# MaaniGhaffari/cvo-rgbd

Hardware: AMD Instinct MI355X
Metric: frame-pair registrations/sec (higher is better)
Workload: dtype f32; 1 GPU; BASELINE configs[1] shape: 64 distinct synthetic 10000x10000 RGB-D cloud pairs (xyz + 5-dim colour) per align_many call, cvo align() to convergence, clouds resident in HBM; points_fixed=10000, points_moving=10000, mode=cvo, batch=64

## Files before the change

cvo-rgbd_amd/csrc/cvo_capi.cpp:

```cpp
#include "cvo_internal.h"

using namespace cvo_dev;
using namespace cvo_impl;

namespace cvo_impl {

int fail(cvo_hip_ctx *ctx, int code, const char *msg)
{
    if (ctx) ctx->err = msg;
    return code;
}

static std::atomic<bool> g_engine_debug{false};
bool engine_debug_on() { return g_engine_debug.load(std::memory_order_relaxed); }

namespace {
struct OptDef {
    const char *key;
    const char *env;
    int env_kind;
    double env_value;
};
const OptDef kOptions[] = {
    {"graph_capture", "CVO_HIP_GRAPH", 1, 1.0},           {"no_graph", "CVO_HIP_NO_GRAPH", 1, 1.0},
    {"head_graphs", "CVO_HIP_RUN_GRAPHS", 1, 1.0},        {"head_mode", "CVO_HIP_NO_HEAD", 1, 0.0},
    {"resident_runs", "CVO_HIP_NO_RUN", 1, 0.0},          {"run_solvers_max", "CVO_HIP_RUN_G_MAX", 2, 0.0},
    {"run_candidates_max", "CVO_HIP_RUN_CAND", 2, 0.0},   {"run_timeout_ms", nullptr, 0, 0.0},
    {"run_fault", nullptr, 0, 0.0},                       {"merged_launches", "CVO_HIP_NO_MERGE", 1, 0.0},
    {"async_builds", "CVO_HIP_NO_ASYNC", 1, 0.0},         {"list_pass_blocks", "CVO_HIP_PROC_BLOCKS", 2, 0.0},
    {"post_debug", "CVO_HIP_POST_DEBUG", 1, 1.0},         {"mailbox_timeout_s", "CVO_HIP_MAILBOX_TIMEOUT_S", 2, 0.0},
    {"candidate_records", "CVO_HIP_NO_CAND", 1, 0.0},     {"sync_upload", "CVO_HIP_SYNC_UPLOAD", 1, 1.0},
    {"engine_debug", "CVO_HIP_ENGINE_DEBUG", 1, 1.0},     {"one_launch_hand_over", "CVO_HIP_NO_CLOUD_ONE", 1, 0.0},
    {"small_calls_alone", "CVO_HIP_NO_ALONE", 1, 0.0},    {"fused_groups", "CVO_HIP_NO_FUSE", 1, 0.0},
    {"engines", "CVO_HIP_ENGINES_FORCE", 2, 0.0},         {"list_init", "CVO_HIP_LIST_INIT", 2, 0.0},
    {"kept_pack", "CVO_HIP_NO_PACK", 1, 0.0},             {"list_margin", "CVO_HIP_LIST_MARGIN", 2, 0.0},
    {"final_mirror", "CVO_HIP_NO_FINAL_MIRROR", 1, 0.0},  {"twist_on_shared_gpu", "CVO_HIP_TWIST_ON_SHARED_GPU", 1, 1.0},
    {"comm_debug", "CVO_HIP_COMM_DEBUG", 1, 1.0},         {"wait_policy", "CVO_HIP_WAIT_POLICY", 2, 0.0},
    {"acvo_runs", "CVO_HIP_NO_ACVO_RUN", 1, 0.0},         {"tail_alone", "CVO_HIP_TAIL_ALONE", 2, 0.0},         {"side_builds", "CVO_HIP_SIDE", 1, 1.0},
    {"run_build_at", "CVO_HIP_RUN_BUILD_AT", 2, 0.0},         {"alone_max", "CVO_HIP_ALONE_MAX", 2, 0.0},
    {"narrow_merge", "CVO_HIP_NARROW_MERGE", 1, 1.0},     {"narrow_blocks", "CVO_HIP_NARROW_BLOCKS", 2, 0.0},
    {"engine_crowd", "CVO_HIP_ENGINE_CROWD", 2, 0.0},     {"engine_merge_max", "CVO_HIP_ENGINE_MERGE_MAX", 2, 0.0},
    {"matches_combine", nullptr, 0, 0.0},                 {"scan_chunk", nullptr, 0, 0.0},
    {"record_narrow", "CVO_HIP_NO_RECORD_NARROW", 1, 0.0}, {"list_stale_max", "CVO_HIP_LIST_STALE_MAX", 2, 0.0},
};
void env_defaults(cvo_hip_ctx *ctx)
{
    for (const OptDef &d : kOptions) {
        if (!d.env) continue;
        const char *e = getenv(d.env);
        if (!e) continue;
        (void)apply_option(ctx, d.key, d.env_kind == 1 ? d.env_value : atof(e));
    }
}
}

int apply_option(cvo_hip_ctx *ctx, const char *key, double v)
{
    auto is = [&](const char *k) { return std::strcmp(key, k) == 0; };
    const bool on = v != 0.0;
    CtxOptions &o = ctx->opt;
    if (is("graph_capture")) { ctx->use_graphs = on && !o.no_graph; if (!ctx->use_graphs) drop_graphs(ctx); }
    else if (is("no_graph")) { o.no_graph = on; if (on) { ctx->use_graphs = false; drop_graphs(ctx); } }
    else if (is("head_graphs")) ctx->head_graphs = on;
    else if (is("head_mode")) ctx->allow_head = on;
    else if (is("resident_runs")) ctx->allow_run = on;
    else if (is("run_solvers_max")) {
        int cus = 0;
        if (hipDeviceGetAttribute(&cus, hipDeviceAttributeMultiprocessorCount, ctx->device) != hipSuccess || cus <= 0) cus = RUN_G + 8;
        ctx->run_g_max = v > 0.0 ? std::max(8, std::min((int)RUN_G, (int)v)) : std::max(8, std::min((int)RUN_G, cus - 8));
    }
    else if (is("run_candidates_max")) { if (v < 0.0) return CVO_HIP_ERR_INVALID; o.run_cand = (int)v; }
    else if (is("run_timeout_ms")) { if (v < 0.0 || v > 6.0e4) return CVO_HIP_ERR_INVALID; o.run_timeout_ms = v; }
    else if (is("run_fault")) { if (v < 0.0) return CVO_HIP_ERR_INVALID; o.run_fault = (int)v; }
    else if (is("merged_launches")) ctx->allow_merge = on;
    else if (is("async_builds")) ctx->allow_async = ctx->allow_async_self = on;
    else if (is("list_pass_blocks")) {
        const int b = (int)v;
        if (b == 0) { ctx->proc_blocks_forced = false; ctx->proc_blocks = ctx->proc_blocks_default = PROC_BLOCKS; }
        else if (b == 64 || b == 128 || b == 256 || b == 512 || b == 1024) { ctx->proc_blocks = ctx->proc_blocks_default = b; ctx->proc_blocks_forced = true; }
        else return CVO_HIP_ERR_INVALID;
    }
    else if (is("post_debug")) o.post_debug = on;
    else if (is("mailbox_timeout_s")) { if (!(v > 0.0)) return CVO_HIP_ERR_INVALID; o.mailbox_timeout_s = v; }
    else if (is("candidate_records")) o.no_cand = !on;
    else if (is("sync_upload")) o.sync_upload = on;
    else if (is("engine_debug")) { o.engine_debug = on; if (on) g_engine_debug.store(true, std::memory_order_relaxed); }
    else if (is("one_launch_hand_over")) o.no_cloud_one = !on;
    else if (is("small_calls_alone")) o.no_alone = !on;
    else if (is("fused_groups")) o.no_fuse = !on;
    else if (is("engines")) { if (v < 0.0 || v > 8.0) return CVO_HIP_ERR_INVALID; o.engines_force = (int)v; }
    else if (is("list_init")) { if (v < 0.0) return CVO_HIP_ERR_INVALID; o.list_init = v; }
    else if (is("kept_pack")) o.no_pack = !on;
    else if (is("matches_combine")) o.matches_combine = on;
    else if (is("scan_chunk")) { if (v < 0.0 || v > (double)SCAN_CHUNK) return CVO_HIP_ERR_INVALID; o.scan_chunk = (int)v; }
    else if (is("list_margin")) { if (v > 4.0) return CVO_HIP_ERR_INVALID; o.list_margin = v < 0.0 ? -1.0f : (float)v; }
    else if (is("record_narrow")) o.record_narrow = on;
    else if (is("list_stale_max")) { if (!(v >= 1.0 && v <= 64.0)) return CVO_HIP_ERR_INVALID; o.list_stale_max = (float)v; }
    else if (is("final_mirror")) o.no_final_mirror = !on;
    else if (is("twist_on_shared_gpu")) o.twist_on_shared_gpu = on;
    else if (is("comm_debug")) o.comm_debug = on;
    else if (is("wait_policy")) { if (v < 0.0 || v > 2.0) return CVO_HIP_ERR_INVALID; o.wait_policy = (int)v; }
    else if (is("acvo_runs")) o.no_acvo_run = !on;
    else if (is("tail_alone")) { if (v < 0.0 || v > 32.0) return CVO_HIP_ERR_INVALID; o.tail_alone = (int)v; }
    else if (is("run_restart")) o.no_restart = !on;
    else if (is("side_builds")) o.no_side_builds = !on;
    else if (is("run_build_at")) { if (!(v > 0.0 && v <= 1.0)) return CVO_HIP_ERR_INVALID; o.run_build_at = (float)v; }
    else if (is("alone_max")) { if (v < 0.0 || v > 64.0) return CVO_HIP_ERR_INVALID; o.alone_max = (int)v; }
    else if (is("narrow_merge")) o.narrow_merge = on;
    else if (is("narrow_blocks")) { const int b = (int)v; if (b != 0 && b != 32 && b != 64) return CVO_HIP_ERR_INVALID; o.narrow_blocks = b; }
    else if (is("engine_crowd")) { if (v < 0.0) return CVO_HIP_ERR_INVALID; o.engine_crowd = (int)std::min(v, 1.0e6); }
    else if (is("engine_merge_max")) { if (v < 0.0 || v > 32.0) return CVO_HIP_ERR_INVALID; o.engine_merge_max = (int)v; }
    else return CVO_HIP_ERR_INVALID;
    return CVO_HIP_OK;
}

const char *params_problem(const cvo_hip_params &p)
{
    if (p.mode != CVO_HIP_MODE_CVO && p.mode != CVO_HIP_MODE_ACVO)
        return "params.mode must be CVO_HIP_MODE_CVO or CVO_HIP_MODE_ACVO (MATLAB: default_params() returns mode CVO)";
    if (p.max_iter < 0) return "params.max_iter < 0";
    const float pos[] = {p.ell_init, p.sigma, p.sp_thres, p.c, p.d, p.c_ell, p.c_sigma};
    const char *pos_name[] = {"ell_init", "sigma", "sp_thres", "c", "d", "c_ell", "c_sigma"};
    static thread_local char msg[96];
    for (int i = 0; i < 7; ++i)
        if (!(pos[i] > 0.0f) || !std::isfinite(pos[i])) {
            snprintf(msg, sizeof(msg), "params.%s must be positive and finite", pos_name[i]);
            return msg;
        }
    if (p.mode == CVO_HIP_MODE_ACVO && (!(p.c_sp_thres > 0.0f) || !std::isfinite(p.c_sp_thres)))
        return "params.c_sp_thres must be positive and finite";
    if (p.mode == CVO_HIP_MODE_ACVO && (!(p.ell_max_init > 0.0f) || !std::isfinite(p.ell_max_init) ||
                                        !(p.ell_min >= 0.0f) || !std::isfinite(p.dl_step)))
        return "params.ell_max_init / ell_min / dl_step out of range";
    const float fin[] = {p.min_step, p.eps, p.eps_2, p.color_scale, p.ell_min};
    for (float v : fin)
        if (!std::isfinite(v)) return "params: min_step, eps, eps_2, color_scale, ell_min must be finite";
    if (p.color_scale < 0.0f) return "params.color_scale < 0";
    return nullptr;
}

DevParams make_dev_params(const cvo_hip_params &p)
{
    DevParams d{};
    d.mode = p.mode;
    d.max_iter = p.max_iter;
    d.ell_init = p.ell_init;
    d.ell_min = p.ell_min;
    d.ell_max_init = p.ell_max_init;
    d.sp = p.sp_thres;
    d.c_sp = (p.mode == CVO_HIP_MODE_ACVO) ? p.c_sp_thres : p.sp_thres;
    d.c = p.c;
    d.d = p.d;
    d.c_ell = p.c_ell;
    d.min_step = p.min_step;
    d.eps = p.eps;
    d.eps_2 = p.eps_2;
    const float s2 = p.sigma * p.sigma;
    const float cs2 = p.c_sigma * p.c_sigma;
    d.log_sp_s2 = (float)std::log((double)(p.sp_thres / s2));
    d.tau_c = (float)(-2.0 * p.c_ell * p.c_ell *
                      (double)(float)std::log((double)(d.c_sp / p.c_sigma / p.c_sigma)));
    d.s2_d = (double)s2;
    d.cs2_d = (double)cs2;
    d.dl_step = p.dl_step;
    d.color_scale = p.color_scale;
    d.build_at = 0.7f;
    d.record_narrow = 1;
    d.list_stale_max = 3.0f;
    d.list_margin = 0.15f;
    return d;
}


}

extern "C" {


const char *cvo_hip_error_string(int status)
{
    switch (status) {
    case CVO_HIP_OK: return "ok";
    case CVO_HIP_ERR_INVALID: return "invalid argument or call order";
    case CVO_HIP_ERR_HIP: return "HIP runtime error";
    case CVO_HIP_ERR_NOMEM: return "out of memory";
    case CVO_HIP_ERR_COMM: return "RCCL / all-reduce error";
    case CVO_HIP_ERR_NODEVICE: return "no usable HIP device";
    case CVO_HIP_ERR_RUN: return "a resident run timed out and the registration could not be redone";
    default: return "unknown status";
    }
}

const char *cvo_hip_last_error(const cvo_hip_ctx *ctx) { return ctx ? ctx->err.c_str() : ""; }

int cvo_hip_device_count(int *count)
{
    if (!count) return CVO_HIP_ERR_INVALID;
    int n = 0;
    if (hipGetDeviceCount(&n) != hipSuccess) n = 0;
    *count = n;
    return CVO_HIP_OK;
}

int cvo_hip_default_params(int mode, cvo_hip_params *p)
{
    if (!p || (mode != CVO_HIP_MODE_CVO && mode != CVO_HIP_MODE_ACVO && mode != CVO_HIP_MODE_MATLAB))
        return CVO_HIP_ERR_INVALID;
    std::memset(p, 0, sizeof(*p));
    p->mode = mode == CVO_HIP_MODE_MATLAB ? CVO_HIP_MODE_CVO : mode;
    p->max_iter = 2000;
    p->sigma = 0.1f;
    p->c = 7.0f;
    p->d = 7.0f;
    p->c_sigma = 1.0f;
    p->min_step = (float)(2 * 1.0e-1);
    p->eps = (float)(5 * 1.0e-5);
    p->eps_2 = (float)1.0e-5;
    if (mode == CVO_HIP_MODE_ACVO) {
        p->ell_init = 0.1f;
        p->ell_min = 0.0391f;
        p->ell_max_init = 0.15f;
        p->sp_thres = 8.315e-3f;
        p->c_sp_thres = 8.315e-3f;
        p->c_ell = 0.5f;
        p->dl_step = 0.3;
    } else {
        p->ell_init = 0.15f;
        p->ell_min = 0.0f;
        p->ell_max_init = 0.15f;
        p->sp_thres = 8e-3f;
        p->c_sp_thres = 8e-3f;
        p->c_ell = 200.0f;
        p->dl_step = 0.0;
    }
    if (mode == CVO_HIP_MODE_MATLAB) {
        p->sp_thres = 1e-3f;
        p->c_sp_thres = 1e-3f;
        p->eps = 5e-4f;
        p->eps_2 = 1e-4f;
        p->color_scale = 1e-5f;
    }
    return CVO_HIP_OK;
}

int cvo_hip_init_state(const cvo_hip_params *p, cvo_hip_state *s)
{
    if (!p || !s) return CVO_HIP_ERR_INVALID;
    std::memset(s, 0, sizeof(*s));
    s->R[0] = s->R[4] = s->R[8] = 1.0f;
    s->ell = p->ell_init;
    s->ell_max = p->ell_max_init;
    for (float *m : {s->transform, s->prev_transform, s->accum_transform})
        m[0] = m[5] = m[10] = m[15] = 1.0f;
    return CVO_HIP_OK;
}

// ... 449 lines not shown
    if (!ctx || !out) return CVO_HIP_ERR_INVALID;
    HIP_TRY(ctx, hipSetDevice(ctx->device));
    const bool had_tf = ctx->have_tf;
    std::swap(ctx->fixed, ctx->scratch_a);
    std::swap(ctx->moving, ctx->scratch_b);
    int rc = upload_cloud(ctx, ctx->fixed, xyz_a, feat_a, na, feat_layout);
    if (!rc) rc = upload_cloud(ctx, ctx->moving, xyz_b, feat_b, nb, feat_layout);
    if (!rc) rc = cvo_hip_function_inner_product(ctx, ell, out);
    std::swap(ctx->fixed, ctx->scratch_a);
    std::swap(ctx->moving, ctx->scratch_b);
    ctx->have_tf = had_tf;
    return rc;
}

int cvo_hip_get_wave_load(cvo_hip_ctx *ctx, uint32_t *members_per_wave, int capacity, int *waves)
{
    cvo_lock::Api api_guard;
    if (!ctx || !members_per_wave || !waves || capacity < 0) return CVO_HIP_ERR_INVALID;
    HIP_TRY(ctx, hipSetDevice(ctx->device));
    const int n = std::min(capacity, 4 * ctx->proc_blocks);
    *waves = 0;
    if (!ctx->kept_cnt.p || n <= 0) return CVO_HIP_OK;
    HIP_TRY(ctx, hipStreamSynchronize(ctx->stream));
    HIP_TRY(ctx, hipMemcpy(members_per_wave, ctx->kept_cnt.p, (size_t)n * sizeof(uint32_t), hipMemcpyDeviceToHost));
    *waves = n;
    return CVO_HIP_OK;
}

int cvo_hip_set_graph_capture(cvo_hip_ctx *ctx, int enable)
{
    cvo_lock::Api api_guard;
    if (!ctx) return CVO_HIP_ERR_INVALID;
    return apply_option(ctx, "graph_capture", enable ? 1.0 : 0.0);
}

int cvo_hip_set_profiling(cvo_hip_ctx *ctx, int enable)
{
    cvo_lock::Api api_guard;
    if (!ctx) return CVO_HIP_ERR_INVALID;
    ctx->profiling = enable != 0;
    return CVO_HIP_OK;
}

int cvo_hip_get_profile(cvo_hip_ctx *ctx, cvo_hip_profile *out, int reset)
{
    cvo_lock::Api api_guard;
    if (!ctx || !out) return CVO_HIP_ERR_INVALID;
    int rc = drain_events(ctx);
    if (rc) return rc;
    *out = ctx->prof;
    if (reset) ctx->prof = cvo_hip_profile{};
    return CVO_HIP_OK;
}

int cvo_hip_get_graph_stats(const cvo_hip_ctx *ctx, long long *launches_from_cache, long long *captures)
{
    if (!ctx || !launches_from_cache || !captures) return CVO_HIP_ERR_INVALID;
    *launches_from_cache = ctx->plans.hits;
    *captures = ctx->plans.captures;
    return CVO_HIP_OK;
}

int cvo_hip_get_run_stats(cvo_hip_ctx *ctx, int *runs, int *declined, int *iterations, int *candidates)
{
    cvo_lock::Api api_guard;
    if (!ctx || !ctx->st) return CVO_HIP_ERR_INVALID;
    struct { int32_t run_count, run_entered, run_iterations, run_candidates; } f{};
    static_assert(offsetof(DevState, run_candidates) - offsetof(DevState, run_count) == 12, "four consecutive words");
    if (hipSetDevice(ctx->device) != hipSuccess || hipStreamSynchronize(ctx->stream) != hipSuccess ||
        hipMemcpy(&f, reinterpret_cast<const char *>(ctx->st) + offsetof(DevState, run_count), sizeof(f), hipMemcpyDeviceToHost) != hipSuccess)
        return CVO_HIP_ERR_HIP;
    if (runs) *runs = f.run_entered;
    if (declined) *declined = f.run_count - f.run_entered;
    if (iterations) *iterations = f.run_iterations;
    if (candidates) *candidates = f.run_candidates;
    return CVO_HIP_OK;
}

int cvo_hip_get_list_stats(const cvo_hip_ctx *ctx, int *builds, int *narrowings, int *reexpansions)
{
    if (!ctx) return CVO_HIP_ERR_INVALID;
    if (builds) *builds = ctx->list_stats[0];
    if (narrowings) *narrowings = ctx->list_stats[1];
    if (reexpansions) *reexpansions = ctx->list_stats[2];
    return CVO_HIP_OK;
}

int cvo_hip_get_run_clocks(cvo_hip_ctx *ctx, long long clocks16[16])
{
    cvo_lock::Api api_guard;
    if (!ctx || !ctx->st || !clocks16) return CVO_HIP_ERR_INVALID;
    long long clk[16];
    static_assert(sizeof(clk) == sizeof(DevState::run_clk), "run_clk");
    if (hipSetDevice(ctx->device) != hipSuccess || hipStreamSynchronize(ctx->stream) != hipSuccess ||
        hipMemcpy(clk, reinterpret_cast<const char *>(ctx->st) + offsetof(DevState, run_clk), sizeof(clk), hipMemcpyDeviceToHost) != hipSuccess)
        return CVO_HIP_ERR_HIP;
    for (int q = 0; q < 16; ++q) clocks16[q] = clk[q];
    return CVO_HIP_OK;
}

int cvo_hip_set_option(cvo_hip_ctx *ctx, const char *key, double value)
{
    cvo_lock::Api api_guard;
    if (!ctx || !key) return CVO_HIP_ERR_INVALID;
    if (hipSetDevice(ctx->device) != hipSuccess) return CVO_HIP_ERR_HIP;
    const int rc = apply_option(ctx, key, value);
    if (rc) return fail(ctx, rc, "cvo_hip_set_option: unknown key or value out of range");
    return CVO_HIP_OK;
}

int cvo_hip_get_option(const cvo_hip_ctx *ctx, const char *key, double *value)
{
    if (!ctx || !key || !value) return CVO_HIP_ERR_INVALID;
    auto is = [&](const char *k) { return std::strcmp(key, k) == 0; };
    const CtxOptions &o = ctx->opt;
    if (is("graph_capture")) *value = ctx->use_graphs;
    else if (is("no_graph")) *value = o.no_graph;
    else if (is("head_graphs")) *value = ctx->head_graphs;
    else if (is("head_mode")) *value = ctx->allow_head;
    else if (is("resident_runs")) *value = ctx->allow_run;
    else if (is("run_solvers_max")) *value = ctx->run_g_max;
    else if (is("run_candidates_max")) *value = o.run_cand;
    else if (is("run_timeout_ms")) *value = o.run_timeout_ms;
    else if (is("run_fault")) *value = o.run_fault;
    else if (is("merged_launches")) *value = ctx->allow_merge;
    else if (is("async_builds")) *value = ctx->allow_async;
    else if (is("list_pass_blocks")) *value = ctx->proc_blocks_forced ? ctx->proc_blocks : 0;
    else if (is("post_debug")) *value = o.post_debug;
    else if (is("mailbox_timeout_s")) *value = o.mailbox_timeout_s;
    else if (is("candidate_records")) *value = !o.no_cand;
    else if (is("sync_upload")) *value = o.sync_upload;
    else if (is("engine_debug")) *value = o.engine_debug;
    else if (is("one_launch_hand_over")) *value = !o.no_cloud_one;
    else if (is("small_calls_alone")) *value = !o.no_alone;
    else if (is("fused_groups")) *value = !o.no_fuse;
    else if (is("engines")) *value = o.engines_force;
    else if (is("narrow_merge")) *value = o.narrow_merge;
    else if (is("narrow_blocks")) *value = o.narrow_blocks;
    else if (is("engine_crowd")) *value = o.engine_crowd;
    else if (is("engine_merge_max")) *value = o.engine_merge_max;
    else if (is("list_init")) *value = o.list_init;
    else if (is("kept_pack")) *value = !o.no_pack;
    else if (is("matches_combine")) *value = o.matches_combine;
    else if (is("scan_chunk")) *value = o.scan_chunk;
    else if (is("list_margin")) *value = o.list_margin;
    else if (is("record_narrow")) *value = o.record_narrow;
    else if (is("list_stale_max")) *value = o.list_stale_max;
    else if (is("final_mirror")) *value = !o.no_final_mirror;
    else if (is("twist_on_shared_gpu")) *value = o.twist_on_shared_gpu;
    else if (is("comm_debug")) *value = o.comm_debug;
    else if (is("wait_policy")) *value = o.wait_policy;
    else if (is("acvo_runs")) *value = !o.no_acvo_run;
    else if (is("tail_alone")) *value = o.tail_alone;
    else if (is("tail_handovers")) *value = (double)ctx->tail_handovers;
    else if (is("run_restart")) *value = !o.no_restart;
    else if (is("side_builds")) *value = !o.no_side_builds;
    else if (is("run_build_at")) *value = o.run_build_at;
    else if (is("side_builds_launched")) *value = (double)ctx->side_builds_launched;
    else if (is("alone_max")) *value = o.alone_max;
    else if (is("run_timeouts")) *value = (double)ctx->run_timeouts;
    else if (is("list_grows")) *value = (double)ctx->list_grows;
    else if (is("async_builds_named")) *value = (double)ctx->async_stats[0];
    else if (is("async_stalls")) *value = (double)ctx->async_stats[1];
    else if (is("run_aborts")) *value = (double)ctx->run_aborts;
    else if (is("engine_begins")) *value = (double)ctx->engine_begins;
    else if (is("engine_final_mirrored")) *value = (double)ctx->engine_final_mirrored;
    else if (is("engine_final_copied")) *value = (double)ctx->engine_final_copied;
    else if (is("no_run_backoff")) *value = ctx->no_run_backoff;
    else return CVO_HIP_ERR_INVALID;
    return CVO_HIP_OK;
}

long long cvo_hip_get_mirror_retries(void) { return mirror_retries().load(std::memory_order_relaxed); }

int cvo_hip_synchronize(cvo_hip_ctx *ctx)
{
    cvo_lock::Api api_guard;
    if (!ctx) return CVO_HIP_ERR_INVALID;
    HIP_TRY(ctx, hipStreamSynchronize(ctx->stream));
    return CVO_HIP_OK;
}


}
```

cvo-rgbd_amd/csrc/cvo_device.h:

```cpp
#pragma once

#include <hip/hip_runtime.h>
#include <hip/hip_ext.h>
#include <stddef.h>
#include <stdint.h>

#include "cvo_hip.h"
#include "se3_math.hpp"

namespace cvo_dev {

constexpr int FEAT_STRIDE = 8;
constexpr int FEAT_INDEX_SLOT = 5;

constexpr int BLOCK = 256;
constexpr int TILES_PER_WAVE = 4;
constexpr int ROWS_PER_WAVE = 16 * TILES_PER_WAVE;
constexpr int ROWS_PER_TILE = 4 * ROWS_PER_WAVE;
constexpr float PAD_BIG = 1.0e30f;
constexpr int PROC_BLOCKS = 1024;
constexpr int PROC_WAVES = PROC_BLOCKS * 4;

constexpr int NSUB = 256;
constexpr int PROC_PARTS = PROC_BLOCKS / NSUB;
constexpr int TILE_STAGE = 128;
constexpr int DEAL_SHIFT = 2;
constexpr int PAIR_QUEUE = 128;
constexpr int SEG = 64;
constexpr int MAX_CSEG = 32;

typedef uint4 TileEntry;

enum ProcMode { PROC_FLOW = 0, PROC_STEP = 1, PROC_SELF = 2 };
enum ListId { LIST_XY = 0, LIST_XX = 1, LIST_YY = 2, LIST_KEPT = 3, LIST_XYB = 4, LIST_XXB = 5, LIST_YYB = 6,
              LIST_N = 7 };
CVO_HD int self_list_id(int l, int buf) { return buf ? LIST_XXB + l : LIST_XX + l; }

constexpr int NACC_FLOW = 9;
constexpr int NACC_STEP = 4;
constexpr int NACC_SELF = 2;
constexpr int NACC_MAX = 9;

constexpr int RED_FLOW = 0, RED_XX = 9, RED_YY = 11, RED_STEP = 13, RED_N = 17;

enum { RUNNING = 0, DONE_BREAK_A = 1, DONE_BREAK_B = 2, DONE_MAX_ITER = 3, NEED_BIGGER_LIST = 4,
       DONE_COMM_ERROR = 5,
       DONE_RUN_TIMEOUT = 6 };

constexpr int MAX_WORLD = 16;
constexpr int MAIL_VALS = 14;
struct alignas(128) MailSlot {
    double v[MAIL_VALS];
    unsigned long long seq;
    unsigned long long pad_;
};
struct Mailbox {
    MailSlot slot[2][MAX_WORLD];
    unsigned long long owner_dev;
    unsigned long long pad_[15];
};
struct CommTable {
    Mailbox *peer[MAX_WORLD];
    int rank, world;
    long long timeout_ticks;
};

constexpr int RUN_G = 248;
constexpr int RUN_G_SMALL = 32;
constexpr int RUN_BLOCK = 512;
constexpr int RUN_WAVES = RUN_BLOCK / 64;
constexpr int RUN_LANES = RUN_G * RUN_BLOCK;
constexpr int RUN_R = 8;
constexpr int RUN_MIRROR_ABORTED = 1 << 29;
constexpr int RUN_MIRROR_ENTERED = 1 << 30;
constexpr int RUN_L = 8;
constexpr int RUN_CAP = RUN_LANES * (RUN_R + RUN_L);
constexpr unsigned RUN_LDS_BYTES = (unsigned)RUN_L * 2u * (unsigned)RUN_BLOCK * 16u;
constexpr int RUN_NV = 13;
#ifndef CVO_RUN_A
#define CVO_RUN_A 4
#endif
constexpr int RUN_A = CVO_RUN_A;
constexpr int RUN_GEN = 4;
constexpr int RUN_CHAINS = 8;
struct RunMail {
    unsigned long long w[RUN_GEN][RUN_G + 1][2 * RUN_NV];
    unsigned long long p[RUN_GEN][RUN_CHAINS][2 * RUN_NV];
    unsigned long long entry_ticket;
    unsigned long long entry_go;
    unsigned long long side_done;
    unsigned long long side_req;
};
constexpr int RUN_G_SIDE = 128;

struct KernConsts {
    float tau;
    float tau_c;
    float sp;
    float inv_c;
    float inv_d;
    float inv_l3;
    float cb, cg, cd;
    float cscale;
    double s2_d;
    double cs2_d;
    double ninv_2l2;
    double ninv_2cl2;
};

struct DevParams {
    int32_t mode, max_iter;
    float ell_init, ell_min, ell_max_init;
    float sp, c_sp;
    float c, d, c_ell;
    float min_step, eps, eps_2;
    float log_sp_s2;
    float tau_c;
    float list_margin;
    int32_t async_xy;
    float build_at;
    int32_t async_self;
    float color_scale;
    float run_cand_cap;
    int32_t record_narrow;
    float list_stale_max;
    double s2_d, cs2_d, dl_step;
};

struct alignas(16) DevHead {
    float R[9], T[3];
    float ell, ell_max;
    float Rt[9], t[3];
    float used_Rt[9], used_t[3];
    KernConsts kc;
    float kc_ell, kc_pad_;
    float center[3];
    float xmax, y0max;
    float tauf[3];
    int32_t n_fixed;
    uint32_t pad0_;
    float list_r[3];
    int32_t list_ok[3];
    int32_t reuse[3];
    int32_t ck_nblk[3];
    float list_Rt[9], list_t[3];
    float rec_r;
    int32_t narrow;
    float rec_Rt[9], rec_t[3];
    int32_t list_stat[3];
    int32_t async_stat[2];
    int32_t rec_pad_;
    int32_t xy_active, xy_target, stall, xy_fresh;
    int32_t xy_ok[2];
    int32_t xy_ck[2];
    float xy_r[2];
    float tauf_build;
    float r_last;
    float xy_Rt[2][9], xy_t[2][3];
    int32_t sf_active[2], sf_target[2], sf_fresh[2];
    int32_t sf_ok[2][2];
    int32_t sf_ck[2][2];
    float sf_r[2][2];
    float sf_tauf_build[2];
    cvo_math::XiConsts xi;
    float omega[3], v[3];
    double dl;
    double red[RED_N];
    int32_t k;
    int32_t done;
    int32_t iter;
    int32_t n_exec;
    int32_t n_slots;
    int32_t pending;
    unsigned long long mail_snap;
    int32_t run_hint;
    int32_t head_check_;
    int32_t rec_count[2];
};
enum { REC_NARROW = 1, REC_BOUNDED = 2 };
CVO_HD unsigned head_check_mix(unsigned x, unsigned y, unsigned z, unsigned w, unsigned piece)
{
    return (x * 0x9E3779B1u + y * 0x85EBCA77u + z * 0xC2B2AE3Du + w * 0x27D4EB2Fu) ^ (piece * 0x165667B1u + 0x9E3779B9u);
}
struct DevState : DevHead {
    uint32_t sub[LIST_N][NSUB];
    uint32_t ovf[2][8];
    uint32_t built[3][64];
    int32_t run_count;
    int32_t run_entered;
    int32_t run_iterations;
    int32_t run_candidates;
    int32_t run_last_entered, run_last_aborted;
    long long run_clk[16];
    unsigned long long mail_seq;
    unsigned long long run_seq;
};
static_assert(LIST_N <= 8, "DevState::ovf holds 8 lists");
constexpr size_t DEVSTATE_INIT_BYTES = offsetof(DevState, mail_seq);
constexpr size_t DEVSTATE_HEAD_BYTES = sizeof(DevHead);
static_assert(offsetof(DevState, sub) == sizeof(DevHead) && sizeof(DevHead) % 16 == 0, "the tail follows the head");

constexpr int MAXG = 16;
template <class A> struct Grp { A a[MAXG]; };
constexpr int ENGINE_SLOTS = 32;

struct FilterArgs {
    const float4 *pos_a;
    const float4 *pos_b;
    const float4 *seg_a;
    const float4 *seg_b;
    DevState *st;
    DevState *st2;
    TileEntry *tiles;
    TileEntry *tiles_b;
    int async_xy;
    uint32_t subcap;
    int list;
    int row_lo, row_hi;
    int nb;
    int jt;
    int tf_a, tf_b;
    int check_done;
    int gx, gy;
    long long *dbg;
    float4 *pos_bt;
};

struct ProcessArgs {
    const float4 *pos_a;
    const float *feat_a;
    const float4 *pos_b;
    const float *feat_b;
    const TileEntry *tiles;
    const TileEntry *tiles_b;
    int async_xy;
    int async_self;
    uint2 *kept_ij;
    float *kept_a;
    uint32_t *kept_cnt;
    double *partials;
    DevState *st;
    DevState *st2;
    uint32_t subcap;
    uint32_t kept_wcap;
    int nblk;
    const double *flow_part;
    const double *xx_part;
    const double *yy_part;
    cvo_hip_trace *trace; int trace_cap;
    int acvo;
    int32_t *done_mirror;
    int list;
    int row_hi, nb;
    int first_counted;
    int tf_a, tf_b;
    int check_done;
    int weight;
    uint2 *cand;
    uint32_t *cand_cnt;
    uint2 *cand_b;
    uint32_t *cand_cnt_b;
    int need_d2;
    const CommTable *comm;
    int kept_packed;
    unsigned kept_ebase;
};

enum { POST_REDUCE = 1, POST_MATH = 2 };

struct PostFlowArgs {
    DevState *st;
    const double *part_flow;
    const double *part_xx;
    const double *part_yy;
    cvo_hip_trace *trace; int trace_cap;
    int flags;
    int check_done;
    int32_t *done_mirror;
    int nblk;
    const CommTable *comm;
    DevParams prm;
};

struct PostStepArgs {
    DevState *st;
    DevState *st2;
    const double *part_step;
    cvo_hip_trace *trace; int trace_cap;
    int flags;
    int check_done;
    long long *dbg;
    int32_t *done_mirror;
    int ck_nblk[3];
    int32_t *progress_mirror;
    int nblk;
    const CommTable *comm;
    DevHead *final_mirror;
    uint32_t *build_mask;
    uint32_t slot_bit;
    RunMail *run_mail;
    int32_t *run_mirror;
    int32_t *hint_mirror;
    int run_iters;
    int run_g_max;
    long long run_timeout_ticks;
    int32_t *side_mirror;
    float run_build_at;
    int run_fault;
    DevParams prm;
};

constexpr size_t kTableHeaderBytes = 256;
constexpr int MAX_OPS = 10;
struct OpArgs {
    ProcessArgs p;
    FilterArgs f;
    union {
        PostFlowArgs pf;
        PostStepArgs ps;
    };
    int np, n0, n1, n2;
};
struct Slot {
    int active;
    int pad_[3];
    OpArgs op[MAX_OPS];
};

CVO_HD KernConsts make_kconsts(const DevParams &p, float ell)
{
    KernConsts k;
    const float l = ell;
    k.tau = (float)(-2.0 * l * l * (double)p.log_sp_s2);
    k.tau_c = p.tau_c;
    k.sp = p.sp;
    k.inv_c = 1 / p.c;
    k.inv_d = 1 / p.d;
    const float ell_3 = l * l * l;
    k.inv_l3 = 1 / ell_3;
    const float temp_coef = (float)(1 / (2.0 * l * l));
    k.cb = (float)(-2.0 * temp_coef);
    k.cg = -temp_coef;
    k.cd = (float)(2.0 * temp_coef);
    k.cscale = p.color_scale;
    if (k.cscale > 0.0f) k.tau = (float)((double)k.tau * 1.00001);
    if (!(k.tau > 0.0f)) k.tau = 0.0f;
    k.s2_d = p.s2_d;
    k.cs2_d = p.cs2_d;
    k.ninv_2l2 = -1.0 / (2.0 * l * l);
    k.ninv_2cl2 = -1.0 / (2.0 * p.c_ell * p.c_ell);
    return k;
}

CVO_HD void compute_filter_bounds(DevHead *s, bool identity)
{
    float ymax = s->y0max;
    if (!identity) {
        const float *R = s->R, *c = s->center;
        float sh2 = 0.0f;
        for (int r = 0; r < 3; ++r) {
            const float rc = R[3 * r] * c[0] + R[3 * r + 1] * c[1] + R[3 * r + 2] * c[2];
            const float d = s->T[r] + rc - c[r];
            sh2 += d * d;
        }
        ymax = (s->y0max + sqrtf(sh2)) * 1.0001f + 1e-6f;
    }
    const float u16 = 16.0f / 16777216.0f;
    const float sxy = (s->xmax + ymax) * (s->xmax + ymax);
    const float sxx = 4.0f * s->xmax * s->xmax;
    const float syy = 4.0f * ymax * ymax;
    const float tau = s->kc.tau;
    s->tauf[LIST_XY] = (tau + u16 * sxy) * 1.000001f;
    s->tauf[LIST_XX] = (tau + u16 * sxx) * 1.000001f;
    s->tauf[LIST_YY] = (tau + u16 * syy) * 1.000001f;
}

CVO_HD bool spheres_near(const float4 sa, const float4 sb, float reach)
{
    const float ex = sa.x - sb.x, ey = sa.y - sb.y, ez = sa.z - sb.z;
    const float d2 = __builtin_fmaf(ez, ez, __builtin_fmaf(ey, ey, ex * ex));
    const float rr = (sa.w + sb.w + reach) * 1.00001f + 1e-5f;
    return d2 * 0.99999f <= rr * rr;
}
CVO_HD float cull_slack(const float *t, const float cx, const float cy, const float cz, const float xmax, const float y0max)
{
    const float W = ((fabsf(cx) + fabsf(cy)) + fabsf(cz)) + (xmax + y0max);
    return (64.0f / 16777216.0f) * (3.0003f * W + ((fabsf(t[0]) + fabsf(t[1])) + fabsf(t[2])));
}

CVO_HD float reuse_slack(const float *t, const float *c, const float xmax, const float y0max, const float sides)
{
    const float W = ((fabsf(c[0]) + fabsf(c[1])) + fabsf(c[2])) + (xmax + y0max);
    const float S = 3.0003f * W + ((fabsf(t[0]) + fabsf(t[1])) + fabsf(t[2]));
    return 1.0e-4f * (1.0f + xmax + y0max) + sides * (22.0f / 16777216.0f) * S;
}

constexpr float LIST_LOOSE = 1.3f;
CVO_HD float pose_travel(const DevHead *s, const float *Rt0, const float *t0, const float ymax)
{
    float f2 = 0.0f, c2 = 0.0f;
    for (int r = 0; r < 3; ++r) {
        float dc = s->t[r] - t0[r];
        for (int q = 0; q < 3; ++q) {
            const float d = s->Rt[3 * r + q] - Rt0[3 * r + q];
            f2 += d * d;
            dc += d * s->center[q];
        }
        c2 += dc * dc;
    }
    return sqrtf(0.5f * f2) * 1.001f * ymax + sqrtf(c2);
}
CVO_HD void plan_lists(DevHead *s, DevHead *bulk, const bool store, const DevParams &p, const float r_now)
{
    const float ymax = s->y0max;
    const float slack_xx = reuse_slack(s->t, s->center, s->xmax, ymax, 0.0f), slack_xy = reuse_slack(s->t, s->center, s->xmax, ymax, 1.0f);
    const float wide_yy = slack_xy - slack_xx;
    const float margin = p.list_margin;
    const bool sync_xy = s->list_ok[LIST_XY] && !p.async_xy;
    const float travel = sync_xy ? pose_travel(s, s->list_Rt, s->list_t, ymax) : 0.0f;
#pragma unroll
    for (int l = 0; l < 3; ++l) {
        if (l == LIST_XY && p.async_xy) continue;
        if (l != LIST_XY && p.async_self) continue;
        if (l != LIST_XY && p.mode != CVO_HIP_MODE_ACVO) { s->reuse[l] = 1; continue; }
        const float slack = l == LIST_XX ? slack_xx : slack_xy;
        const float need = (r_now + (l == LIST_XY ? travel : 0.0f)) * 1.0001f + slack;
        const float lr = s->list_r[l];
        const float r0 = r_now * 1.0001f + slack;
        const float rb = r0 * (1.0f + margin);
        bool keep = margin > 0.0f && s->list_ok[l] && need <= lr;
        if (l == LIST_XY && p.record_narrow && keep && s->ck_nblk[LIST_XY] != 0) {
            const float tr = pose_travel(s, s->rec_Rt, s->rec_t, ymax);
            const float rr = s->rec_r;
            keep = (r_now + tr) * 1.0001f + slack <= rr && lr <= fmaxf(p.list_stale_max, LIST_LOOSE) * (1.0f + margin) * r0;
            s->narrow &= REC_BOUNDED;
            if (keep && !(rr <= LIST_LOOSE * (1.0f + margin) * r0)) {
                keep = (rb + tr) * 1.0001f + slack <= rr;
                if (keep) {
                    s->rec_r = rb * 1.000001f;
                    s->narrow = REC_NARROW | REC_BOUNDED;
                    s->list_stat[1] += 1;
                    if (store) {
                        for (int q = 0; q < 9; ++q) bulk->rec_Rt[q] = s->Rt[q];
                        for (int q = 0; q < 3; ++q) bulk->rec_t[q] = s->t[q];
                    }
                }
            }
        } else {
            keep = keep && lr <= LIST_LOOSE * (1.0f + margin) * r0;
            if (l == LIST_XY) s->narrow &= REC_BOUNDED;
        }
        s->reuse[l] = keep ? 1 : 0;
        if (keep) continue;
        s->ck_nblk[l] = 0;
        s->list_r[l] = rb * 1.000001f;
        s->list_ok[l] = 1;
        if (margin > 0.0f) {
            const float rw = s->list_r[l] + (l == LIST_YY ? wide_yy : 0.0f);
            s->tauf[l] = (rw * rw + (s->tauf[l] - s->kc.tau)) * 1.000001f;
        }
        if (l == LIST_XY) {
            s->rec_r = s->list_r[l];
            s->narrow = p.record_narrow ? REC_BOUNDED : 0;
            s->list_stat[0] += 1;
            if (store) {
                for (int q = 0; q < 9; ++q) bulk->list_Rt[q] = bulk->rec_Rt[q] = s->Rt[q];
                for (int q = 0; q < 3; ++q) bulk->list_t[q] = bulk->rec_t[q] = s->t[q];
            }
        }
    }
}

template <int B> CVO_HD float xy_travel(const DevHead *s, const DevHead *rec)
{
    float f2 = 0.0f, c2 = 0.0f;
    for (int r = 0; r < 3; ++r) {
        float dc = s->t[r] - rec->xy_t[B][r];
        for (int q = 0; q < 3; ++q) {
// ... 469 lines not shown
```

cvo-rgbd_amd/csrc/cvo_engine.cpp:

```cpp
#include "cvo_internal.h"

using namespace cvo_dev;
using namespace cvo_impl;

namespace cvo_impl {

bool fusable(const cvo_hip_ctx *c) { return !c->profiling && !multi_rank(c) && !(c->prm.color_scale > 0.0f); }



struct EngineProfile {
    std::mutex mu;
    bool on = false;
    double flow_ms = 0.0, flow_slots = 0.0;
    long long flow_launches = 0;
    std::vector<float> dur_us, period_us;
    std::vector<int> slots;
};
EngineProfile *engine_profile()
{
    static EngineProfile *p = new EngineProfile;
    return p;
}

bool better_alone(const std::deque<AlignJob *> &pending)
{
    const bool off = !pending.empty() && pending.front()->ctx->opt.no_alone;
    if (off || engine_profile()->on) return false;
    double pairs = 0.0;
    bool acvo = false;
    for (const AlignJob *j : pending) {
        const cvo_hip_ctx *c = j->ctx;
        acvo = c->prm.mode == CVO_HIP_MODE_ACVO;
        if (!c->allow_head || !c->allow_async || !c->allow_merge || c->opt.no_cand || c->fixed.np > 65536 || c->moving.np > 65536 ||
            (acvo ? !c->allow_async_self : !c->allow_run))
            return false;
        pairs = std::max(pairs, (double)c->fixed.n * (double)c->moving.n);
    }
    const size_t few = acvo ? (pairs <= 1.6e7 ? 12 : (pairs <= 5.0e7 ? 4 : (pairs <= 1.2e8 ? 4 : 0)))
                            : (pairs <= 1.6e7 ? 12 : (pairs <= 5.0e7 ? 8 : (pairs <= 2.0e8 ? 4 : 0)));
    if (const int force = pending.front()->ctx->opt.alone_max) return pending.size() <= (size_t)force;
    return pending.size() <= few;
}

struct Engine {
    int device = 0;
    hipStream_t s = nullptr;
    TableBuf tab;
    PlanCache plans;
    bool in_use = false;

    AlignJob *member[ENGINE_SLOTS] = {};
    std::vector<RecOp> ops[ENGINE_SLOTS];
    Slot slot[ENGINE_SLOTS];
    struct Retire { hipEvent_t ev = nullptr; std::vector<AlignJob *> jobs; };
    std::vector<Retire> retiring;
    hipEvent_t ev[4] = {};
    std::vector<PrepareEntry> prep;
    long long launched = 0, checked = 0;
    int zdim = 0;
    bool crowded = true, use_graph = true, dirty = true, failed = false;
    int batch_len = kEngineBatch;
    bool narrow = false;
    bool narrow_merge = false;
    int narrow_blocks = 0;
    bool wind_down = false;
    std::vector<TLaunch> plan;
    struct FlowEv { hipEvent_t a, b; int live; };
    std::vector<FlowEv> flow_ev;
    long long n_batches[5] = {}, n_replans = 0, n_inserts = 0, n_sends = 0, n_prepares = 0, n_mirrored = 0, n_copied = 0;
    double t_replan = 0, t_insert = 0, t_launch = 0, t_finish = 0, t_wait = 0, t_collect = 0, t_idle_at = 0;
    static double now_ms() { return std::chrono::duration<double, std::milli>(std::chrono::steady_clock::now().time_since_epoch()).count(); }

    int create(int dev)
    {
        device = dev;
        if (hipSetDevice(dev) != hipSuccess) return -1;
        if (hipStreamCreateWithFlags(&s, hipStreamNonBlocking) != hipSuccess) return -1;
        if (tab.init(ENGINE_SLOTS, s) != 0) return -1;
        for (auto &e : ev)
            if (hipEventCreateWithFlags(&e, hipEventDisableTiming) != hipSuccess) return -1;
        return 0;
    }

    int live() const { int n = 0; for (AlignJob *j : member) n += j != nullptr; return n; }
    bool idle() const { return live() == 0 && retiring.empty() && launched == checked; }

    static int nblk_for(int z)
    {
        constexpr int budget = 2048;
        int nblk = 64;
        while (nblk < PROC_BLOCKS && nblk * 2 <= (budget + z / 2) / std::max(1, z)) nblk *= 2;
        return nblk;
    }

    void finish_job(AlignJob *j, int rc)
    {
        j->rc = rc;
        j->phase = 2;
        j->in_group = false;
        j->ctx->loop_stream = nullptr;
        j->ctx->crowded = false;
        j->ctx->lone = true;
        j->ctx->proc_blocks = j->ctx->proc_blocks_default;
    }

    void fail_all(const char *msg, std::deque<AlignJob *> &pending)
    {
        failed = true;
        (void)hipStreamSynchronize(s);
        for (AlignJob *&j : member)
            if (j) { finish_job(j, fail(j->ctx, CVO_HIP_ERR_HIP, msg)); j = nullptr; }
        for (auto &r : retiring) {
            for (AlignJob *j : r.jobs) finish_job(j, fail(j->ctx, CVO_HIP_ERR_HIP, msg));
            if (r.ev) (void)hipEventDestroy(r.ev);
        }
        retiring.clear();
        for (AlignJob *j : pending) { j->rc = fail(j->ctx, CVO_HIP_ERR_HIP, msg); j->phase = 2; }
        pending.clear();
        prep.clear();
        for (int z = 0; z < ENGINE_SLOTS; ++z) slot[z].active = 0;
        (void)tab.sync(slot, s, 0);
        (void)hipStreamSynchronize(s);
        launched = checked = 0;
    }

    int flush_prepare()
    {
        if (prep.empty()) return CVO_HIP_OK;
        launch_prepare_many(prep.data(), (int)prep.size(), s, tab.masks());
        n_prepares += ((long long)prep.size() + MAXG - 1) / MAXG;
        prep.clear();
        return hipGetLastError() == hipSuccess ? CVO_HIP_OK : CVO_HIP_ERR_HIP;
    }

    int insert(AlignJob *j, int z)
    {
        cvo_hip_ctx *c = j->ctx;
        c->loop_stream = s;
        c->crowded = crowded;
        c->lone = false;
        j->in_group = true;
        int rc = CVO_HIP_OK;
        if (j->phase == 3) {
            int32_t zero = 0;
            std::memcpy(&c->st_host[kPollSlots].done, &zero, sizeof(zero));
            if (hipMemcpyAsync(reinterpret_cast<char *>(c->st) + offsetof(DevState, done), &c->st_host[kPollSlots].done,
                               sizeof(zero), hipMemcpyHostToDevice, s) != hipSuccess)
                rc = fail(c, CVO_HIP_ERR_HIP, "resume failed");
            *c->done_mirror = 0;
            PrepareEntry e{};
            e.st = c->st;
            e.prm = loop_params(c);
            if (!rc) prep.push_back(e);
            j->phase = 0;
        } else {
            PrepareEntry e{};
            rc = job_begin(*j, &e);
            if (!rc) prep.push_back(e);
        }
        if (rc) { finish_job(j, rc); return rc; }
        ++c->engine_begins;
        if (j->phase != 0) {
            Retire r;
            if (flush_prepare() != CVO_HIP_OK ||
                hipMemcpyAsync(&c->st_host[0], c->st, sizeof(DevState), hipMemcpyDeviceToHost, s) != hipSuccess ||
                hipEventCreateWithFlags(&r.ev, hipEventDisableTiming) != hipSuccess || hipEventRecord(r.ev, s) != hipSuccess) {
                if (r.ev) (void)hipEventDestroy(r.ev);
                finish_job(j, fail(c, CVO_HIP_ERR_HIP, "event failed"));
                return CVO_HIP_ERR_HIP;
            }
            r.jobs.push_back(j);
            retiring.push_back(r);
            return CVO_HIP_OK;
        }
        member[z] = j;
        ops[z].clear();
        dirty = true;
        return CVO_HIP_OK;
    }

    int replan()
    {
        int n = 0;
        for (int z = 0; z < ENGINE_SLOTS; ++z) n += member[z] != nullptr;
        int zd = 1;
        while (zd < n) zd *= 2;
        if (n > 16 && n <= 24) zd = 24;
        for (int z = ENGINE_SLOTS - 1, hole = 0; z >= zd; --z) {
            if (!member[z]) continue;
            while (member[hole]) ++hole;
            member[hole] = member[z]; member[z] = nullptr;
            ops[hole].swap(ops[z]); ops[z].clear();
        }
        const bool regeom = zd != zdim;
        zdim = zd;
        const int nblk = (narrow && narrow_blocks > 0) ? std::min(narrow_blocks, nblk_for(zdim)) : nblk_for(zdim);
        int merge_max = 2;
        std::vector<const std::vector<RecOp> *> po;
        std::vector<Slot *> ps;
        for (int z = 0; z < ENGINE_SLOTS; ++z)
            if (member[z]) { merge_max = member[z]->ctx->opt.engine_merge_max; break; }
        for (int z = 0; z < ENGINE_SLOTS; ++z) {
            if (!member[z]) { slot[z].active = 0; continue; }
            cvo_hip_ctx *c = member[z]->ctx;
            if (regeom || ops[z].empty()) {
                c->proc_blocks = nblk;
                const bool allow = c->allow_merge;
                if (zdim > merge_max && !(narrow && narrow_merge)) c->allow_merge = false;
                const int rc = record_iteration(c, ops[z], 0);
                c->allow_merge = allow;
                if (rc) return rc;
            }
            std::memset(&slot[z], 0, sizeof(Slot));
            slot[z].active = 1;
            po.push_back(&ops[z]);
            ps.push_back(&slot[z]);
        }
        if (!plan_fused(po, ps, zdim, plan)) return CVO_HIP_ERR_INVALID;
        for (int z = 0; z < ENGINE_SLOTS; ++z)
            if (member[z]) set_build_masks(slot[z], plan, tab.masks(), z);
        const int nq = po.empty() ? 0 : (int)po[0]->size();
        if (tab.sync(slot, s, nq) != 0) return CVO_HIP_ERR_HIP;
        ++n_replans;
        dirty = false;
        return CVO_HIP_OK;
    }

    void collect_stopped()
    {
        Retire r;
        for (int z = 0; z < ENGINE_SLOTS; ++z) {
            AlignJob *j = member[z];
            if (!j) continue;
            cvo_hip_ctx *c = j->ctx;
            const int32_t verdict = *(volatile int32_t *)c->done_mirror;
            if (verdict == RUNNING) continue;
            const bool mirrored = (verdict == DONE_BREAK_A || verdict == DONE_BREAK_B || verdict == DONE_MAX_ITER) && c->final_mirror &&
                                  !c->opt.no_final_mirror && !multi_rank(c);
            if (mirrored && take_final_mirror(c, verdict)) {
                ++n_mirrored;
                ++c->engine_final_mirrored;
                finish_job(j, job_finish(*j));
            } else if (hipMemcpyAsync(&j->ctx->st_host[0], j->ctx->st, sizeof(DevState), hipMemcpyDeviceToHost, s) != hipSuccess) {
                finish_job(j, fail(j->ctx, CVO_HIP_ERR_HIP, "state copy failed"));
            } else {
                ++n_copied;
                ++c->engine_final_copied;
                r.jobs.push_back(j);
            }
            member[z] = nullptr;
            ops[z].clear();
            dirty = true;
        }
        if (r.jobs.empty()) return;
        if (hipEventCreateWithFlags(&r.ev, hipEventDisableTiming) != hipSuccess || hipEventRecord(r.ev, s) != hipSuccess) {
            for (AlignJob *j : r.jobs) finish_job(j, fail(j->ctx, CVO_HIP_ERR_HIP, "event failed"));
            if (r.ev) (void)hipEventDestroy(r.ev);
            return;
        }
        retiring.push_back(r);
    }

    bool finish_arrived(std::deque<AlignJob *> &pending, bool block)
    {
        bool moved = false;
        while (!retiring.empty()) {
            Retire &r = retiring.front();
            const hipError_t q = block ? hipEventSynchronize(r.ev) : hipEventQuery(r.ev);
            if (q == hipErrorNotReady) break;
            block = false;
            for (AlignJob *j : r.jobs) {
                cvo_hip_ctx *c = j->ctx;
                const DevState &cur = c->st_host[0];
                if (q != hipSuccess) { finish_job(j, fail(c, CVO_HIP_ERR_HIP, "state event failed")); continue; }
                if (cur.done != NEED_BIGGER_LIST) { finish_job(j, job_finish(*j)); continue; }
                int rc = CVO_HIP_OK;
                for (int l = 0; l < LIST_N && !rc; ++l)
                    if (cur.ovf[0][l] | cur.ovf[1][l]) {
                        uint32_t worst = 0;
                        for (int qq = 0; qq < NSUB; ++qq) worst = std::max(worst, cur.sub[l][qq]);
                        const double grown = std::min(
                            4.0e9, std::max((double)worst * NSUB, (double)c->lists[l].cap) * 1.5 + 1024.0);
                        rc = ensure_list(c, l, 0, 0, grown);
                        ++c->list_grows;
                    }
                for (int qq = 0; qq < 3 && !rc; ++qq) {
                    const int la = qq == 0 ? LIST_XY : (qq == 1 ? LIST_XX : LIST_YY), lb = qq == 0 ? LIST_XYB : (qq == 1 ? LIST_XXB : LIST_YYB);
                    if (!c->lists[la].cap && !c->lists[lb].cap) continue;
                    const double both = (double)std::max(c->lists[la].cap, c->lists[lb].cap);
                    rc = ensure_list(c, la, 0, 0, both);
                    if (!rc && c->lists[lb].cap) rc = ensure_list(c, lb, 0, 0, both);
                }
                if (rc) { finish_job(j, rc); continue; }
                j->executed_base = cur.k;
                j->phase = 3;
                pending.push_front(j);
            }
            (void)hipEventDestroy(r.ev);
            retiring.erase(retiring.begin());
            moved = true;
        }
        return moved;
    }

    int launch_one_batch()
    {
        const int batch = batch_len;
        if (engine_profile()->on) {
            for (int k = 0; k < batch; ++k)
                for (const TLaunch &l : plan) {
                    if (l.kernel == TK_FLOW || l.kernel == TK_FLOW_D2) {
                        FlowEv fe{nullptr, nullptr, live()};
                        if (hipEventCreate(&fe.a) == hipSuccess && hipEventCreate(&fe.b) == hipSuccess) {
                            launch_table(tab.dev, l, s, fe.a, fe.b);
                            flow_ev.push_back(fe);
                            continue;
                        }
                    }
                    launch_table(tab.dev, l, s);
                }
            return hipGetLastError() == hipSuccess ? CVO_HIP_OK : CVO_HIP_ERR_HIP;
        }
        return run_plan(tab.dev, plans, plan, s, use_graph, batch);
    }

    bool pump(std::deque<AlignJob *> &pending, int want)
    {
        if (failed) return false;
        if (hipSetDevice(device) != hipSuccess) { fail_all("hipSetDevice failed", pending); return true; }
        bool moved = false;
        while (checked < launched) {
            const hipError_t q = hipEventQuery(ev[checked % 4]);
            if (q == hipErrorNotReady) break;
            if (q != hipSuccess) { fail_all("fused poll failed", pending); return true; }
            ++checked;
            { const double t0 = now_ms(); collect_stopped(); t_collect += now_ms() - t0; }
            moved = true;
        }
        { const double t0 = now_ms(); if (finish_arrived(pending, false)) moved = true; t_finish += now_ms() - t0; }
        while (!wind_down && !pending.empty() && live() < std::min(want, (int)ENGINE_SLOTS)) {
            AlignJob *j = pending.front();
            pending.pop_front();
            int z = 0;
            while (member[z]) ++z;
            { const double t0 = now_ms(); insert(j, z); t_insert += now_ms() - t0; }
            moved = true;
        }
        {
            const double t0 = now_ms();
            const int rc = flush_prepare();
            t_insert += now_ms() - t0;
            if (rc) { fail_all("prepare launch failed", pending); return true; }
        }
        constexpr long long depth = 2;
        while (live() > 0 && launched - checked < depth && !wind_down) {
            if (dirty) {
                const double t0 = now_ms();
                const int rc = replan();
                t_replan += now_ms() - t0;
                if (rc) { fail_all("fused launch recording failed", pending); return true; }
            }
            const double t_l0 = now_ms();
            const int rc_launch = launch_one_batch();
            if (rc_launch != CVO_HIP_OK ||
                hipEventRecord(ev[launched % 4], s) != hipSuccess) {
                fail_all("fused launch failed", pending);
                return true;
            }
            t_launch += now_ms() - t_l0;
            ++launched;
            ++n_batches[zdim >= 16 ? 4 : (zdim >= 8 ? 3 : (zdim >= 4 ? 2 : (zdim >= 2 ? 1 : 0)))];
            moved = true;
        }
        if (live() == 0 && dirty && launched == checked) {
            if (replan() != CVO_HIP_OK) { fail_all("table update failed", pending); return true; }
        }
        return moved;
    }

    void release_members(std::vector<AlignJob *> &out)
    {
        if (!wind_down || launched != checked || failed) return;
        collect_stopped();
        for (int z = 0; z < ENGINE_SLOTS; ++z) {
            AlignJob *j = member[z];
            if (!j) continue;
            out.push_back(j);
            member[z] = nullptr;
            ops[z].clear();
            dirty = true;
        }
    }

    void wait_oldest(std::deque<AlignJob *> &pending)
    {
        const double t0 = now_ms();
        struct Acc { double &t; double t0; ~Acc() { t += now_ms() - t0; } } acc{t_wait, t0};
        if (checked < launched) {
            if (hipEventSynchronize(ev[checked % 4]) != hipSuccess) fail_all("fused poll failed", pending);
        } else if (!retiring.empty()) {
            (void)hipEventSynchronize(retiring.front().ev);
        }
    }
};

std::mutex *engine_mutex()
{
    static std::mutex *mu = new std::mutex;
    return mu;
}

Engine *engine_checkout(int device)
{
    static std::vector<Engine *> *all = new std::vector<Engine *>();
    std::lock_guard<std::mutex> lock(*engine_mutex());
    for (Engine *e : *all)
        if (!e->in_use && e->device == device && !e->failed) { e->in_use = true; return e; }
    size_t have = 0;
    for (Engine *e : *all) have += e->device == device && !e->failed;
    Engine *first = nullptr;
    for (size_t k = have; k < std::max<size_t>(have + 1, 4); ++k) {
        Engine *e = new (std::nothrow) Engine();
        if (!e) break;
        if (e->create(device) != 0) { (void)hipGetLastError(); delete e; break; }
        all->push_back(e);
        if (!first) first = e;
    }
    if (first) first->in_use = true;
    return first;
}

void engine_release(Engine *e)
{
    if (!e->flow_ev.empty()) {
        EngineProfile *pr = engine_profile();
        std::lock_guard<std::mutex> plock(pr->mu);
        for (size_t q = 0; q < e->flow_ev.size(); ++q) {
            auto &fe = e->flow_ev[q];
            float ms = 0.f, gap = 0.f;
            if (hipEventSynchronize(fe.b) == hipSuccess && hipEventElapsedTime(&ms, fe.a, fe.b) == hipSuccess) {
                pr->flow_ms += ms; pr->flow_launches++; pr->flow_slots += fe.live;
                if (q + 1 < e->flow_ev.size() && hipEventElapsedTime(&gap, fe.a, e->flow_ev[q + 1].a) != hipSuccess) gap = 0.f;
                if (pr->dur_us.size() < (size_t)1 << 20) {
                    pr->dur_us.push_back(ms * 1e3f); pr->period_us.push_back(gap * 1e3f); pr->slots.push_back(fe.live);
                }
            }
        }
        for (auto &fe : e->flow_ev) {
            (void)hipEventDestroy(fe.a);
            (void)hipEventDestroy(fe.b);
        }
        e->flow_ev.clear();
    }
    std::lock_guard<std::mutex> lock(*engine_mutex());
    if (engine_debug_on())
        fprintf(stderr, "[cvo_hip] engine %p: batches at zdim 1/2/4/8/16: %lld %lld %lld %lld %lld, replans %lld, "
                "prepare launches %lld, final states mirrored %lld copied %lld, graph captures %lld hits %lld; host ms: insert %.2f replan %.2f launch %.2f collect %.2f finish %.2f wait %.2f\n",
                (void *)e, e->n_batches[0], e->n_batches[1], e->n_batches[2],
                e->n_batches[3], e->n_batches[4], e->n_replans, e->n_prepares, e->n_mirrored, e->n_copied, e->plans.captures, e->plans.hits,
                e->t_insert, e->t_replan, e->t_launch, e->t_collect, e->t_finish, e->t_wait);
    e->t_insert = e->t_replan = e->t_launch = e->t_collect = e->t_finish = e->t_wait = 0;
    for (long long &v : e->n_batches) v = 0;
    e->n_replans = e->n_prepares = e->n_mirrored = e->n_copied = 0;
    e->launched = e->checked = 0;
    e->in_use = false;
}


}

extern "C" {

int cvo_hip_align_many(cvo_hip_ctx **ctxs, cvo_hip_state **states, int *n_iters, int count)
{
    cvo_lock::Api api_guard;
    if (count < 0 || (count > 0 && (!ctxs || !states))) return CVO_HIP_ERR_INVALID;
    const bool dbg_many = engine_debug_on();
    const double t_many0 = Engine::now_ms();
    struct Tell { double t0; int n; ~Tell() { if (engine_debug_on()) fprintf(stderr, "[cvo_hip] align_many(%d): %.2f ms\n", n, Engine::now_ms() - t0); } } tell{t_many0, count};
    std::vector<AlignJob> jobs((size_t)count);
    for (int i = 0; i < count; ++i) {
        if (!ctxs[i] || !states[i]) return CVO_HIP_ERR_INVALID;
        for (int k = 0; k < i; ++k)
            if (ctxs[k] == ctxs[i]) return CVO_HIP_ERR_INVALID;
        jobs[i].ctx = ctxs[i];
        jobs[i].s = states[i];
        jobs[i].n_iter = n_iters ? &n_iters[i] : nullptr;
    }
    int first_err = CVO_HIP_OK;
    std::vector<char> taken((size_t)count, 0);
    std::vector<AlignJob *> leavers;
    const bool no_fuse = count > 0 && ctxs[0] && ctxs[0]->opt.no_fuse;
    if (!no_fuse && count > 1) {
        constexpr int gmax = ENGINE_SLOTS;
        for (int i = 0; i < count; ++i) {
            if (taken[i] || jobs[i].phase != 0 || !fusable(jobs[i].ctx)) continue;
            std::deque<AlignJob *> pending;
            for (int k = i; k < count; ++k)
                if (!taken[k] && jobs[k].phase == 0 && fusable(jobs[k].ctx) &&
                    jobs[k].ctx->device == jobs[i].ctx->device &&
                    jobs[k].ctx->prm.mode == jobs[i].ctx->prm.mode)
                    pending.push_back(&jobs[k]);
            if (pending.size() < 2) continue;
            if (better_alone(pending)) continue;
            for (AlignJob *j : pending) taken[j - &jobs[0]] = 1;
            const size_t total = pending.size();
            constexpr size_t max_engines = 4;
            size_t ngroups = total > 3 * ENGINE_SLOTS ? 4 : (total >= 40 ? 3 : (total >= 8 ? 2 : 1));
            ngroups = std::max<size_t>(1, std::min(ngroups, max_engines));
            if (const int force = pending.front()->ctx->opt.engines_force) ngroups = (size_t)std::max(1, std::min(force, 8));
            bool graphs_ok = true;
            for (AlignJob *j : pending) graphs_ok = graphs_ok && j->ctx->use_graphs;
            const int crowd = pending.front()->ctx->opt.engine_crowd;
            std::vector<Engine *> engines;
            for (size_t g = 0; g < ngroups; ++g) {
                Engine *e = engine_checkout(jobs[i].ctx->device);
                if (!e) break;
                e->crowded = (int)total > crowd;
                e->use_graph = graphs_ok;
                e->zdim = 0;
                e->wind_down = false;
                e->narrow = false;
                e->narrow_merge = pending.front()->ctx->opt.narrow_merge;
                e->narrow_blocks = pending.front()->ctx->opt.narrow_blocks;
                e->batch_len = kEngineBatch;
                e->t_idle_at = 0;
                e->dirty = true;
                engines.push_back(e);
            }
            if (engines.empty()) {
                for (AlignJob *j : pending) taken[j - &jobs[0]] = 0;
                continue;
            }
            const int share = std::min<int>(gmax, (int)((total + engines.size() - 1) / engines.size()));
            const int tail_k = pending.empty() ? 0 : pending.front()->ctx->opt.tail_alone;
            const int narrow_from = pending.empty() ? 0 : (pending.front()->ctx->prm.mode == CVO_HIP_MODE_ACVO ? 8 : 24);
            bool tail_ok = tail_k > 0 && !engine_profile()->on;
            for (AlignJob *j : pending) {
                const cvo_hip_ctx *c = j->ctx;
                tail_ok = tail_ok && c->allow_head && c->allow_async && c->allow_merge && !c->opt.no_cand && runs_allowed(c) && c->fixed.np <= 65536 &&
                          c->moving.np <= 65536 && (c->prm.mode == CVO_HIP_MODE_CVO || (c->allow_async_self && !c->opt.no_acvo_run)) &&
                          (double)c->fixed.n * (double)c->moving.n <= 2.0e8;
            }
            const bool narrow_merge_ok = !pending.empty() && (pending.front()->ctx->opt.narrow_merge || pending.front()->ctx->opt.narrow_blocks > 0) && !engine_profile()->on;
            int dbg_left = -1, dbg_narrow = -1;
            for (;;) {
                bool any = false, moved = false;
                if ((tail_ok || narrow_merge_ok) && pending.empty() && !engines.front()->wind_down) {
                    int left = 0;
                    bool narrow = true, settled = true;
                    for (Engine *e : engines) {
                        settled = settled && e->retiring.empty();
                        for (AlignJob *j : e->member)
                            if (j) { ++left; narrow = narrow && *(volatile int32_t *)j->ctx->progress_mirror >= narrow_from; }
                    }
                    if (narrow_merge_ok && narrow && left > 0 && !engines.front()->narrow)
                        for (Engine *e : engines) {
                            e->narrow = true;
                            e->dirty = true;
                            for (int z = 0; z < ENGINE_SLOTS; ++z) e->ops[z].clear();
                        }
                    if (dbg_many && (left != dbg_left || (int)narrow != dbg_narrow)) { dbg_left = left; dbg_narrow = (int)narrow; fprintf(stderr, "[cvo_hip]   %.2f ms: %d left (narrow %d settled %d)\n", Engine::now_ms() - t_many0, left, (int)narrow, (int)settled); }
                    (void)settled;
                    if (tail_ok && left > 0 && left <= tail_k && narrow) {
                        for (Engine *e : engines) e->wind_down = true;
                        if (dbg_many) {
                            fprintf(stderr, "[cvo_hip]   tail: %d registrations left after %.2f ms, slots done:", left, Engine::now_ms() - t_many0);
                            for (Engine *e : engines)
                                for (AlignJob *j : e->member)
                                    if (j) fprintf(stderr, " %d", *(volatile int32_t *)j->ctx->progress_mirror);
                            fprintf(stderr, "\n");
                        }
                    }
                }
                for (Engine *e : engines) {
                    if (e->wind_down) {
                        const size_t before = leavers.size();
                        e->release_members(leavers);
                        if (leavers.size() != before) {
                            moved = true;
                            if (dbg_many) fprintf(stderr, "[cvo_hip]   tail: %zu registrations leave engine %p after %.2f ms\n", leavers.size() - before, (void *)e, Engine::now_ms() - t_many0);
                        }
                        while (!pending.empty()) {
                            leavers.push_back(pending.front());
                            pending.pop_front();
                            moved = true;
                        }
                    }
                    if (e->pump(pending, share)) moved = true;
                    if (!e->idle()) any = true;
                    else if (dbg_many && e->t_idle_at == 0) {
                        e->t_idle_at = Engine::now_ms();
                        fprintf(stderr, "[cvo_hip]   engine %p idle after %.2f ms\n", (void *)e, e->t_idle_at - t_many0);
                    }
                }
                if (!any && pending.empty()) break;
                bool alive = false;
                for (Engine *e : engines) alive = alive || !e->failed;
                if (!alive) break;
                if (!moved)
                    for (Engine *e : engines)
                        if (!e->idle() && !e->failed) { e->wait_oldest(pending); break; }
            }
            for (Engine *e : engines) { e->wind_down = false; e->narrow = false; e->batch_len = kEngineBatch; engine_release(e); }
        }
        for (int i = 0; i < count; ++i)
            if (jobs[i].phase == 2 && jobs[i].rc && !first_err) first_err = jobs[i].rc;
    }
    std::vector<char> cont((size_t)count, 0);
    for (AlignJob *j : leavers) {
        const size_t i = (size_t)(j - &jobs[0]);
        taken[i] = 0;
        cont[i] = 1;
    }
    int k_alone = 0;
    for (int i = 0; i < count; ++i)
        if (!taken[i] && jobs[i].phase != 2) ++k_alone;
    const int kAloneLive = std::max<int>(8, (int)leavers.size());
    std::vector<char> begun((size_t)count, 0);
    auto begin_job = [&](int i) {
        int cus = 0;
        if (hipDeviceGetAttribute(&cus, hipDeviceAttributeMultiprocessorCount, jobs[i].ctx->device) != hipSuccess || cus <= 0) cus = RUN_G + 8;
        const int share = std::min(k_alone, kAloneLive);
        jobs[i].ctx->run_g_call = share > 1 ? std::max(8, (cus - 8) / share - 1) : RUN_G;
        jobs[i].ctx->call_no_spec = share > 2;
        jobs[i].ctx->crowded = false;
        jobs[i].ctx->lone = true;
        jobs[i].paced_nb = true;
        begun[(size_t)i] = 1;
        const int rc = cont[(size_t)i] ? job_continue_alone(jobs[i]) : job_begin(jobs[i]);
        if (rc) { jobs[i].rc = rc; jobs[i].phase = 2; if (!first_err) first_err = rc; }
    };
    auto is_alone = [&](int i) { return !taken[i]; };
    for (;;) {
        int live = 0, moved = 0, first_live = -1, waiting = 0;
        for (int i = 0; i < count; ++i)
            if (is_alone(i) && begun[(size_t)i] && jobs[i].phase != 2) ++live;
        for (int i = 0; i < count; ++i)
            if (is_alone(i) && !begun[(size_t)i] && jobs[i].phase != 2 && (live < kAloneLive || multi_rank(jobs[i].ctx))) {
                begin_job(i); ++moved;
                if (jobs[i].phase != 2) ++live;
            }
        live = 0;
        for (int i = 0; i < count; ++i) {
            if (jobs[i].phase == 2) continue;
            if (is_alone(i) && !begun[(size_t)i]) { ++waiting; continue; }
            const int before_phase = jobs[i].phase, before_checked = jobs[i].checked + jobs[i].batches;
            if (job_pump(jobs[i], false)) {
                if (jobs[i].rc && !first_err) first_err = jobs[i].rc;
                ++moved;
                continue;
            }
            ++live;
            if (first_live < 0) first_live = i;
            if (jobs[i].phase != before_phase || jobs[i].checked + jobs[i].batches != before_checked) ++moved;
        }
        if (live == 0 && waiting == 0) break;
        if (!moved && first_live >= 0) {
            if (job_pump(jobs[first_live], true) && jobs[first_live].rc && !first_err)
                first_err = jobs[first_live].rc;
        }
    }
    return first_err;
}

int cvo_hip_engine_profiling(int enable)
{
    EngineProfile *pr = engine_profile();
    std::lock_guard<std::mutex> lock(pr->mu);
    pr->on = enable != 0;
    return CVO_HIP_OK;
}

int cvo_hip_get_engine_profile(double *flow_ms, long long *flow_launches, double *flow_registrations, int reset)
{
    if (!flow_ms || !flow_launches || !flow_registrations) return CVO_HIP_ERR_INVALID;
    EngineProfile *pr = engine_profile();
    std::lock_guard<std::mutex> lock(pr->mu);
    *flow_ms = pr->flow_ms; *flow_launches = pr->flow_launches; *flow_registrations = pr->flow_slots;
    if (reset) { pr->flow_ms = 0.0; pr->flow_launches = 0; pr->flow_slots = 0.0; pr->dur_us.clear(); pr->period_us.clear(); pr->slots.clear(); }
    return CVO_HIP_OK;
}

int cvo_hip_get_engine_flow_trace(float *dur_us, float *period_us, int *slots, int capacity, int *count, int reset)
{
    if (!count || capacity < 0) return CVO_HIP_ERR_INVALID;
    EngineProfile *pr = engine_profile();
    std::lock_guard<std::mutex> lock(pr->mu);
    const int n = (int)std::min<size_t>(pr->dur_us.size(), (size_t)capacity);
    for (int q = 0; q < n; ++q) {
        if (dur_us) dur_us[q] = pr->dur_us[(size_t)q];
        if (period_us) period_us[q] = pr->period_us[(size_t)q];
        if (slots) slots[q] = pr->slots[(size_t)q];
    }
    *count = (int)pr->dur_us.size();
    if (reset) { pr->dur_us.clear(); pr->period_us.clear(); pr->slots.clear(); }
    return CVO_HIP_OK;
}


}
```

cvo-rgbd_amd/csrc/cvo_internal.h:

```cpp
#pragma once
#include "cvo_hip.h"

#include <hip/hip_runtime.h>

#include <algorithm>
#include <atomic>
#include <chrono>
#include <cmath>
#include <cstddef>
#include <cstdint>
#include <cstdio>
#include <cstdlib>
#include <cstring>
#include <deque>
#include <memory>
#include <mutex>
#include <new>
#include <string>
#include <thread>
#include <vector>

#include "cvo_cloud.h"
#include "cvo_comm.h"
#include "cvo_device.h"
// ... 39 lines not shown
};

struct FilterPlan {
    dim3 grid;
    int jt = 0;
};

struct DevBuf {
    void *p = nullptr;
    size_t bytes = 0;
};

struct PinBuf {
    void *p = nullptr;
    size_t bytes = 0;
};

struct List {
    DevBuf a, b;
    uint32_t cap = 0;
};

constexpr int kEngineBatch = 10;
constexpr int kBatch = 8;

constexpr int kStage = 4;
struct TableBuf {
    Slot *dev = nullptr;
    char *raw = nullptr;
    int nslots = 0;
    std::vector<Slot> image;
    Slot *stage = nullptr;
    hipEvent_t stage_ev[kStage] = {};
    bool stage_used[kStage] = {};
    int next = 0;

    int init(int n, hipStream_t s)
    {
        if (dev) return 0;
        if (hipMalloc((void **)&raw, kTableHeaderBytes + (size_t)n * sizeof(Slot)) != hipSuccess) { raw = nullptr; return -1; }
        dev = reinterpret_cast<Slot *>(raw + kTableHeaderBytes);
        if (hipMemsetAsync(raw, 0, kTableHeaderBytes + (size_t)n * sizeof(Slot), s) != hipSuccess) return -1;
        if (arm(s) != 0) return -1;
        if (hipHostMalloc((void **)&stage, (size_t)kStage * n * sizeof(Slot), hipHostMallocDefault) != hipSuccess) return -1;
        for (int i = 0; i < kStage; ++i)
            if (hipEventCreateWithFlags(&stage_ev[i], hipEventDisableTiming) != hipSuccess) return -1;
        nslots = n;
        image.assign((size_t)n, Slot{});
        return 0;
    }
    void destroy()
    {
        for (int i = 0; i < kStage; ++i)
            if (stage_ev[i]) (void)hipEventDestroy(stage_ev[i]);
        if (stage) (void)hipHostFree(stage);
        if (raw) (void)hipFree(raw);
        dev = nullptr; raw = nullptr; stage = nullptr; nslots = 0;
        image.clear();
    }
    uint32_t *masks() const { return reinterpret_cast<uint32_t *>(raw); }
    int arm(hipStream_t s) { return hipMemsetAsync(raw, 0xff, 4 * sizeof(uint32_t), s) == hipSuccess ? 0 : -1; }
    int sync(const Slot *want, hipStream_t s, int nq = MAX_OPS)
    {
        const size_t head = offsetof(Slot, op);
        int lo = nslots, hi = -1;
        for (int z = 0; z < nslots; ++z) {
            const Slot &img = image[(size_t)z];
            bool same = std::memcmp(&img, &want[z], head) == 0;
            if (same && want[z].active) same = std::memcmp(img.op, want[z].op, (size_t)nq * sizeof(OpArgs)) == 0;
            if (!same) { lo = std::min(lo, z); hi = z; }
        }
        if (hi < 0) return 0;
        const int b = next;
        next = (next + 1) % kStage;
        if (stage_used[b] && hipEventSynchronize(stage_ev[b]) != hipSuccess) return -1;
        Slot *st = stage + (size_t)b * nslots;
        const size_t n = (size_t)(hi - lo + 1);
        for (int z = lo; z <= hi; ++z) {
            if (want[z].active) image[(size_t)z] = want[z];
            else image[(size_t)z].active = 0;
            st[z] = image[(size_t)z];
        }
        if (hipMemcpyAsync(&dev[lo], &st[lo], n * sizeof(Slot), hipMemcpyHostToDevice, s) != hipSuccess) return -1;
        if (arm(s) != 0) return -1;
        if (hipEventRecord(stage_ev[b], s) != hipSuccess) return -1;
        stage_used[b] = true;
        return 0;
    }
};

struct PlanGraph {
    std::vector<TLaunch> pre;
    std::vector<TLaunch> plan;
    int iterations = 0;
    hipGraph_t graph = nullptr;
    hipGraphExec_t exec = nullptr;
    uint64_t stamp = 0;
};
struct PlanCache {
    std::vector<PlanGraph> graphs;
    uint64_t clock = 0;
    long long hits = 0, captures = 0;
    int fails = 0;
    void drop()
    {
        for (auto &g : graphs) {
            if (g.exec) (void)hipGraphExecDestroy(g.exec);
            if (g.graph) (void)hipGraphDestroy(g.graph);
        }
        graphs.clear();
    }
};
constexpr int kPollSlots = 4;
constexpr int kEvProcFlow = 10, kEvProcStep = 11;
constexpr int kProcStepTwist = 100;
constexpr int kFlowBuild = 101;
constexpr int kFilterAhead = 102;

struct RecOp {
    enum Kind { FILTER, PROCESS, POST_FLOW, POST_STEP } kind;
    int mode = 0;
    FilterArgs f{};
    ProcessArgs p{};
    PostFlowArgs pf{};
    PostStepArgs ps{};
};


}

using namespace cvo_dev;
using namespace cvo_impl;

struct CtxOptions {
    bool no_cand = false;
    bool no_graph = false;
    bool sync_upload = false;
    bool engine_debug = false;
    bool no_cloud_one = false;
    bool no_alone = false;
    bool no_fuse = false;
    bool no_pack = false;
    bool matches_combine = true;
    int scan_chunk = 0;
    bool no_final_mirror = false;
    bool twist_on_shared_gpu = false;
    bool comm_debug = false;
    bool post_debug = false;
    bool no_side_builds = true;
    float run_build_at = 0.6f;
    bool no_restart = false;
    bool no_acvo_run = false;
    int tail_alone = 8;
    int alone_max = 0;
    int engines_force = 0;
    int narrow_blocks = 0;
    bool narrow_merge = false;
    int engine_crowd = 2;
    int engine_merge_max = 2;
    double list_init = 0.0;
    float list_margin = -1.0f;
    bool record_narrow = true;
    float list_stale_max = 3.0f;
    int run_cand = 0;
    double mailbox_timeout_s = 5.0;
    double run_timeout_ms = 0.0;
    int run_fault = 0;
    int wait_policy = 0;
};

struct cvo_hip_ctx {
    CtxOptions opt;
    int no_run_backoff = 0;
    long long side_builds_launched = 0;
    long long tail_handovers = 0;
    long long engine_begins = 0;
    long long engine_final_mirrored = 0;
    long long engine_final_copied = 0;
    long long run_aborts = 0;
    int list_stats[3] = {0, 0, 0};
    int async_stats[2] = {0, 0};
    long long list_grows = 0;
    long long run_timeouts = 0;
    int device = 0;
    hipStream_t stream = nullptr;
    bool own_stream = false;
    cvo_hip_params prm{};
    DevParams dprm{};
    Cloud fixed, moving;
    Cloud scratch_a, scratch_b;
    DevState *st = nullptr;
    DevHead *st2 = nullptr;
    bool head_mode = false;
    bool allow_head = true;
    DevState *st_host = nullptr;
    int32_t *done_mirror = nullptr;
    int32_t *progress_mirror = nullptr;
    DevHead *final_mirror = nullptr;
    int32_t *run_mirror = nullptr;
    int32_t *hint_mirror = nullptr;
    int32_t *side_mirror = nullptr;
    hipStream_t side_stream = nullptr;
    std::vector<TLaunch> plan_side;
    DevBuf run_mail;
    bool plan_has_final_mirror = false;
    bool allow_run = true;
    int run_g_max = RUN_G;
    int run_g_call = RUN_G;
    bool call_no_spec = false;
    int big_run_backoff = 0;
    bool spec_first_run = true;
    bool head_graphs = false;
    int run_small_max = 0;
    int run_nnz_max = 0;
    std::vector<TLaunch> plan_pre;
    std::vector<RecOp> *rec = nullptr;
    int proc_blocks = PROC_BLOCKS;
    int proc_blocks_default = PROC_BLOCKS;
    bool proc_blocks_forced = false;
    DevBuf raw_xyz, raw_feat;
    DevBuf sort_keys[2], sort_idx[2], sort_tmp;
    float *bbox_dev = nullptr;
    float *bbox_host = nullptr;
    FilterArgs xy_build{};
    bool have_xy_build = false;
    bool allow_async = true;
    bool crowded = false;
    DevBuf cand[3], cand_cnt[3];
    DevBuf cand_xyb, cand_cnt_xyb;
    DevBuf cand_sfb[2], cand_cnt_sfb[2];
    int ck_nblk[3] = {0, 0, 0};
    DevBuf pos_bt;
    bool lone = true;
    bool allow_async_self = true;
    bool use_async_self = false;
    bool use_async = false;
    bool in_loop = false;
    bool plan_recording = false;
    bool merge_twist = false;
    bool allow_merge = true;
    cvo_hip_trace *cur_trace = nullptr;
    int cur_trace_cap = 0;
    hipEvent_t poll_ev[kPollSlots]{};
    DevBuf part_flow, part_xx, part_yy, part_step;
    DevBuf part_hess;
    DevBuf part_score;
    struct ScorePin *score_pin = nullptr;
    DevBuf part_matches;
    PinBuf match_stage;
    DevBuf scan_dev;
    PinBuf scan_stage;
    List lists[LIST_N];
    DevBuf kept_cnt;
    cvo_hip_trace *trace_dev = nullptr;
    int trace_dev_cap = 0;
    bool have_tf = false;
    int row_lo = 0, row_hi = -1, srow_lo = 0, srow_hi = -1;
    bool sharded = false;
    cvo_comm *comm = nullptr;
    Mailbox *mailbox = nullptr;
    CommTable *comm_table = nullptr;
    void *mail_opened[MAX_WORLD] = {};
    int mail_rank = 0, mail_world = 0;
    bool mail_shared_device = false;
    unsigned long long mail_dev_id = 0;
    bool mail_broken = false;
    cvo_hip_allreduce_fn user_allreduce = nullptr;
    void *user_allreduce_arg = nullptr;
    bool profiling = false;
    long long *post_dbg = nullptr;
    TableBuf table;
    PlanCache plans;
    std::vector<TLaunch> plan;
    hipStream_t loop_stream = nullptr;
    bool warm = false;
    bool use_graphs = true;
    int iter_tag = -1;
    std::vector<EventPair> events;
    cvo_hip_profile prof{};
    std::string err;
};

namespace cvo_impl {

#define HIP_TRY(ctx, expr)                                                                   \
    do {                                                                                     \
        hipError_t e_ = (expr);                                                              \
        if (e_ != hipSuccess) {                                                              \
            if (ctx) (ctx)->err = std::string(#expr) + ": " + hipGetErrorString(e_);         \
            return CVO_HIP_ERR_HIP;                                                          \
        }                                                                                    \
    } while (0)

struct AlignJob {
    cvo_hip_ctx *ctx = nullptr;
    cvo_hip_state *s = nullptr;
    cvo_hip_trace *trace = nullptr;
    int trace_cap = 0;
    int *n_iter = nullptr;
    int enq = 0;
    int batches = 0;
    int checked = 0;
    int executed_base = 0;
    int phase = 0;
    int rc = CVO_HIP_OK;
    bool in_group = false;
    int runs_enq = 0;
    bool run_waiting = false;
    bool spec_pending = false;
    bool paced_nb = false;
    int idle_seen = 0;
    int side_seen = 0;
    int side_launched = 0;
    int restarts = 0;
    bool paced = false;
};

int fail(cvo_hip_ctx *ctx, int code, const char *msg);
bool engine_debug_on();
int apply_option(cvo_hip_ctx *ctx, const char *key, double value);
inline bool runs_allowed(const cvo_hip_ctx *ctx) { return ctx->allow_run && ctx->no_run_backoff <= 0; }
const char *params_problem(const cvo_hip_params &p);
DevParams make_dev_params(const cvo_hip_params &p);
int cloud_ready(cvo_hip_ctx *ctx, Cloud &c);
int cloud_reserve(cvo_hip_ctx *ctx, Cloud &c, const float *xyz, const float *feat, int n, int layout);
int upload_cloud(cvo_hip_ctx *ctx, Cloud &c, const float *xyz, const float *feat, int n, int layout, bool on_device = false);
FilterPlan plan_filter(int nrows, int nb);
int ensure_buf(cvo_hip_ctx *ctx, DevBuf &b, size_t bytes);
// ... 50 lines not shown
```

cvo-rgbd_amd/csrc/cvo_job.cpp:

```cpp
#include "cvo_internal.h"

using namespace cvo_dev;
using namespace cvo_impl;

namespace cvo_impl {

void decide_scheme(cvo_hip_ctx *ctx)
{
    const bool small_pair = (double)ctx->fixed.n * (double)ctx->moving.n <= 2.5e7;
    if (!ctx->proc_blocks_forced)
        ctx->proc_blocks = ctx->proc_blocks_default = small_pair ? PROC_BLOCKS / 2 : PROC_BLOCKS;
    ctx->use_async = ctx->allow_async && !ctx->crowded && !ctx->profiling && !multi_rank(ctx) &&
                     !(ctx->prm.color_scale > 0.0f) &&
                     (double)ctx->fixed.n * (double)ctx->moving.n <= 2.0e8;
    ctx->use_async_self = ctx->use_async && ctx->allow_async_self && ctx->lone &&
                          ctx->prm.mode == CVO_HIP_MODE_ACVO;
    const double npairs = (double)ctx->fixed.n * (double)ctx->moving.n;
    if (ctx->use_async_self && !ctx->proc_blocks_forced)
        ctx->proc_blocks = ctx->proc_blocks_default = npairs <= 6.0e7 ? PROC_BLOCKS / 8 : PROC_BLOCKS / 4;
    if (!ctx->proc_blocks_forced && !ctx->use_async_self && ctx->use_async && ctx->lone && ctx->allow_head &&
        ctx->prm.mode == CVO_HIP_MODE_CVO)
    {
        const bool runs = runs_allowed(ctx) && ctx->fixed.np <= 65536 && ctx->moving.np <= 65536;
        ctx->proc_blocks = ctx->proc_blocks_default =
// ... 160 lines not shown
    ctx->run_small_max = 3 * RUN_G_SMALL * RUN_BLOCK;
    if (ctx->prm.mode == CVO_HIP_MODE_ACVO) {
        ctx->run_nnz_max = (int)(0.8 * g_call * RUN_BLOCK * RUN_A);
        ctx->run_small_max = (int)(0.8 * 2 * RUN_G_SMALL * RUN_BLOCK);
    }
    if (ctx->opt.run_cand > 0) ctx->run_nnz_max = ctx->opt.run_cand;
    j.phase = 0;
    ++ctx->tail_handovers;
    return CVO_HIP_OK;
}

int job_finish(AlignJob &j)
{
    cvo_hip_ctx *ctx = j.ctx;
    cvo_hip_state *s = j.s;
    const DevState &f = ctx->st_host[0];
    ctx->have_tf = false;
    if (f.done == DONE_COMM_ERROR) {
        ctx->mail_broken = true;
        if (ctx->opt.comm_debug)
            fprintf(stderr, "[cvo_hip] rank %d of %d: exchange timed out at iteration k = %d (executed %d), mail_seq %llu, mail_snap %llu, slots %d, twist in launch %d\n",
                    ctx->mail_rank, ctx->mail_world, f.k, f.n_exec, (unsigned long long)f.mail_seq, (unsigned long long)f.mail_snap, f.n_slots,
                    (int)(ctx->plan.size() == 4));
        return fail(ctx, CVO_HIP_ERR_COMM, "mailbox all-reduce timed out: a peer rank never delivered its partial sums "
                                           "(the mailboxes must be created and connected again on every rank)");
    }
    if (f.done == DONE_RUN_TIMEOUT)
        return fail(ctx, CVO_HIP_ERR_RUN, "a resident run timed out and the registration could not be redone without runs");
    if (f.done == RUNNING || f.done == NEED_BIGGER_LIST)
        return fail(ctx, CVO_HIP_ERR_INVALID, "align loop ended without a verdict");
    const int executed = f.n_exec;
    for (int q = 0; q < 3; ++q) ctx->list_stats[q] = f.list_stat[q];
    for (int q = 0; q < 2; ++q) ctx->async_stats[q] = f.async_stat[q];
    if (j.trace_cap > 0 && executed > 0)
        HIP_TRY(ctx, hipMemcpy(j.trace, ctx->trace_dev,
                               (size_t)std::min(executed, j.trace_cap) * sizeof(cvo_hip_trace),
                               hipMemcpyDeviceToHost));
    if (executed > 0) cvo_math::tf_to_mat4(f.used_Rt, f.used_t, s->transform);
    std::memcpy(s->R, f.R, sizeof(s->R));
    std::memcpy(s->T, f.T, sizeof(s->T));
    s->ell = f.ell;
    s->ell_max = f.ell_max;
    s->iter = f.iter;
    std::memcpy(s->prev_transform, s->transform, sizeof(s->transform));
    cvo_math::mat4_mul(s->accum_transform, s->transform, s->accum_transform);
    float Rt[9], t[3];
    cvo_math::inverse_tf(s->R, s->T, Rt, t);
    cvo_math::tf_to_mat4(Rt, t, s->transform);
    if (j.n_iter) *j.n_iter = executed;
    if (ctx->profiling) return drain_events(ctx, executed, &f);
    return CVO_HIP_OK;
}

int job_pump(AlignJob &j, bool block)
{
    cvo_hip_ctx *ctx = j.ctx;
    if (j.phase == 2) return 1;
    auto finish_with = [&](int rc) { j.rc = rc; j.phase = 2; return 1; };
    if (hipSetDevice(ctx->device) != hipSuccess) return finish_with(CVO_HIP_ERR_HIP);
    if (j.phase == 0 && (block || j.paced_nb) && (j.paced || j.paced_nb) && !host_reduce(ctx) && !ctx->profiling) {
        const int limit = (ctx->use_async ? 3 : 1) * ctx->prm.max_iter + 4 * kBatch;
        unsigned spins = 0;
        int idle_seen = 0;
        const auto t_enter = std::chrono::steady_clock::now();
        for (;;) {
            if (*(volatile int32_t *)ctx->done_mirror != RUNNING) break;
            const int runs_word = *(volatile int32_t *)ctx->run_mirror;
            const int runs = runs_word & (RUN_MIRROR_ABORTED - 1);
            const int slots = *(volatile int32_t *)ctx->progress_mirror;
            if (!ctx->plan_side.empty()) {
                const int want = *(volatile int32_t *)ctx->side_mirror;
                if (want != 0 && want != j.side_seen) {
                    j.side_seen = want;
                    for (const TLaunch &l : ctx->plan_side) launch_table(ctx->table.dev, l, ctx->side_stream);
                    if (hipGetLastError() != hipSuccess) return finish_with(fail(ctx, CVO_HIP_ERR_HIP, "launching a side build failed"));
                    ++j.side_launched;
                    ++ctx->side_builds_launched;
                }
            }
            const int lead = ctx->head_mode ? 2 : 0;
            bool go;
            if (j.run_waiting) {
                go = runs >= j.runs_enq;
                if (go) {
                    if (runs_word & RUN_MIRROR_ABORTED) { ctx->big_run_backoff = kBigRunBackoff; ++ctx->run_aborts; }
                    else if (j.spec_pending) ctx->spec_first_run = (runs_word & RUN_MIRROR_ENTERED) != 0;
                    j.spec_pending = false;
                    j.enq = slots + kRunBatchSlots; j.run_waiting = false;
                }
            } else {
                go = j.enq - slots <= lead;
            }
            if (go) {
                if (j.enq >= limit) break;
                const int hint = *(volatile int32_t *)ctx->hint_mirror;
                const bool run_plan_ = ctx->head_mode && !ctx->plan_pre.empty();
                const bool first_choice = run_plan_ && j.batches == 1 && j.enq == kShortBatch && j.runs_enq == 0;
                if (run_plan_ && j.batches == 2 && j.runs_enq == 0 && !ctx->spec_first_run && hint > 0) ctx->spec_first_run = hint <= ctx->run_nnz_max;
                const bool big_ok = ctx->big_run_backoff <= 0;
                const bool spec = first_choice && ctx->spec_first_run && big_ok && !ctx->call_no_spec;
                if (spec) j.spec_pending = true;
                const bool with_run = run_plan_ && (spec || (hint > 0 && hint <= (big_ok ? ctx->run_nnz_max : ctx->run_small_max)));
                const bool near_run = ctx->head_mode && !ctx->plan_pre.empty() && !with_run;
                const bool small_run = with_run && !spec && hint > 0 && hint <= ctx->run_small_max;
                const bool two_runs = with_run && !spec && !ctx->plan_side.empty() && hint > 0 &&
                                      hint <= (int)((ctx->prm.mode == CVO_HIP_MODE_ACVO ? 0.8 : 1.0) * RUN_G_SIDE * RUN_BLOCK * 3);
                const int rc = launch_batch(ctx, j.executed_base + j.enq, j.trace_cap, with_run, near_run ? kShortBatch : kBatch, small_run, two_runs);
                if (rc) return finish_with(rc);
                if (with_run) { j.runs_enq += two_runs ? 2 : 1; j.run_waiting = true; }
                else j.enq += near_run ? kShortBatch : kBatch;
                ++j.batches;
                spins = 0;
                idle_seen = 0;
                j.idle_seen = 0;
                if (!j.paced) return 0;
            } else {
                if (!j.paced) {
                    if (!block) return 0;
                    if (std::chrono::steady_clock::now() - t_enter > std::chrono::microseconds(30)) {
                        const hipError_t q = hipStreamQuery(loop_stream(ctx));
                        if (q != hipSuccess && q != hipErrorNotReady)
                            return finish_with(fail(ctx, CVO_HIP_ERR_HIP, "the stream of the align loop reports an error"));
                        if (q == hipSuccess && *(volatile int32_t *)ctx->done_mirror == RUNNING &&
                            *(volatile int32_t *)ctx->progress_mirror == slots && *(volatile int32_t *)ctx->run_mirror == runs_word) {
                            if (++j.idle_seen >= 2)
                                return finish_with(fail(ctx, CVO_HIP_ERR_HIP, "the align loop's stream went idle without progress"));
                        } else {
                            j.idle_seen = 0;
                        }
                        return 0;
                    }
                    __builtin_ia32_pause();
                    continue;
                }
                if (ctx->opt.wait_policy == 0) __builtin_ia32_pause();
                else if (ctx->opt.wait_policy == 1) std::this_thread::yield();
                else std::this_thread::sleep_for(std::chrono::microseconds(50));
                if ((++spins & (ctx->opt.wait_policy == 0 ? 0x3fffu : (ctx->opt.wait_policy == 1 ? 0x3ffu : 0x7u))) == 0u) {
                    const hipError_t q = hipStreamQuery(loop_stream(ctx));
                    if (q != hipSuccess && q != hipErrorNotReady)
                        return finish_with(fail(ctx, CVO_HIP_ERR_HIP, "the stream of the align loop reports an error"));
                    if (q == hipSuccess && *(volatile int32_t *)ctx->done_mirror == RUNNING &&
                        *(volatile int32_t *)ctx->progress_mirror == slots && *(volatile int32_t *)ctx->run_mirror == runs_word) {
                        if (++idle_seen >= 2)
                            return finish_with(fail(ctx, CVO_HIP_ERR_HIP, "the align loop's stream went idle without progress"));
                    } else {
                        idle_seen = 0;
                    }
                }
            }
        }
        {
            const int32_t verdict = *(volatile int32_t *)ctx->done_mirror;
            const bool mirrored = (verdict == DONE_BREAK_A || verdict == DONE_BREAK_B || verdict == DONE_MAX_ITER) && ctx->final_mirror &&
                                  ctx->table.image.size() == 1 && ctx->plan_has_final_mirror;
            if (mirrored && take_final_mirror(ctx, verdict)) return finish_with(job_finish(j));
        }
        if (hipMemcpyAsync(&ctx->st_host[0], ctx->st, sizeof(DevState), hipMemcpyDeviceToHost,
                           ctx->stream) != hipSuccess ||
            hipEventRecord(ctx->poll_ev[0], ctx->stream) != hipSuccess)
            return finish_with(fail(ctx, CVO_HIP_ERR_HIP, "state copy failed"));
        j.phase = 1;
    }
    if (j.phase == 0) {
        bool stop = false;
        while (j.batches - j.checked < 2) {
            int rc = launch_batch(ctx, j.executed_base + j.enq, j.trace_cap);
            if (rc) return finish_with(rc);
            j.enq += kBatch;
            const int slot = j.batches % kPollSlots;
            if (host_reduce(ctx) &&
                hipMemcpyAsync(&ctx->st_host[slot], ctx->st, DEVSTATE_HEAD_BYTES, hipMemcpyDeviceToHost,
                               ctx->stream) != hipSuccess)
                return finish_with(fail(ctx, CVO_HIP_ERR_HIP, "poll copy failed"));
            if (hipEventRecord(ctx->poll_ev[slot], ctx->stream) != hipSuccess)
                return finish_with(fail(ctx, CVO_HIP_ERR_HIP, "poll event failed"));
            ++j.batches;
        }
        const int slot = j.checked % kPollSlots;
        hipError_t q = block ? hipEventSynchronize(ctx->poll_ev[slot]) : hipEventQuery(ctx->poll_ev[slot]);
        if (q == hipErrorNotReady) return 0;
        if (q != hipSuccess) return finish_with(fail(ctx, CVO_HIP_ERR_HIP, "poll event failed"));
        ++j.checked;
        if (host_reduce(ctx) ? ctx->st_host[slot].done != RUNNING
                             : *(volatile int32_t *)ctx->done_mirror != RUNNING)
            stop = true;
        if (j.enq >= (ctx->use_async ? 3 : 1) * ctx->prm.max_iter + 4 * kBatch) stop = true;
        if (!stop) return 0;
        if (hipMemcpyAsync(&ctx->st_host[0], ctx->st, sizeof(DevState), hipMemcpyDeviceToHost,
                           ctx->stream) != hipSuccess ||
            hipEventRecord(ctx->poll_ev[0], ctx->stream) != hipSuccess)
            return finish_with(fail(ctx, CVO_HIP_ERR_HIP, "state copy failed"));
        j.phase = 1;
    }
    hipError_t q = block ? hipEventSynchronize(ctx->poll_ev[0]) : hipEventQuery(ctx->poll_ev[0]);
    if (q == hipErrorNotReady) return 0;
    if (q != hipSuccess) return finish_with(fail(ctx, CVO_HIP_ERR_HIP, "state event failed"));
    const DevState &cur = ctx->st_host[0];
    if (ctx->opt.comm_debug)
        fprintf(stderr, "[cvo_hip] final state: done %d, side mirror %d (seen %d, launched %d), plan_side %zu\n", cur.done, *(volatile int32_t *)ctx->side_mirror,
                j.side_seen, j.side_launched, ctx->plan_side.size());
    if (cur.done == DONE_RUN_TIMEOUT && j.restarts == 0 && !j.in_group && !ctx->opt.no_restart) {
        ++ctx->run_timeouts;
        ++j.restarts;
        ctx->no_run_backoff = kNoRunBackoff + 1;
        const unsigned long long seq = cur.run_seq + 4096ull;
        if ((ctx->side_stream && hipStreamSynchronize(ctx->side_stream) != hipSuccess) || hipStreamSynchronize(loop_stream(ctx)) != hipSuccess ||
            hipMemcpy(reinterpret_cast<char *>(ctx->st) + offsetof(DevState, run_seq), &seq, sizeof(seq), hipMemcpyHostToDevice) != hipSuccess)
            return finish_with(fail(ctx, CVO_HIP_ERR_RUN, "a resident run timed out and the state could not be reset"));
        const int rc = job_begin(j);
        if (rc) return finish_with(rc);
        return 0;
    }
    if (cur.done != NEED_BIGGER_LIST) return finish_with(job_finish(j));
    int rc = CVO_HIP_OK;
    if (ctx->profiling) rc = drain_events(ctx, cur.k + 1, &cur);
    j.executed_base = cur.k;
    for (int l = 0; l < LIST_N && !rc; ++l)
        if (cur.ovf[0][l] | cur.ovf[1][l]) {
            uint32_t worst = 0;
            for (int qq = 0; qq < NSUB; ++qq) worst = std::max(worst, cur.sub[l][qq]);
            const double grown =
                std::min(4.0e9, std::max((double)worst * NSUB, (double)ctx->lists[l].cap) * 1.5 + 1024.0);
            rc = ensure_list(ctx, l, 0, 0, grown);
            ++ctx->list_grows;
        }
    for (int q = 0; q < 3 && !rc; ++q) {
        const int la = q == 0 ? LIST_XY : (q == 1 ? LIST_XX : LIST_YY), lb = q == 0 ? LIST_XYB : (q == 1 ? LIST_XXB : LIST_YYB);
        if (!ctx->lists[la].cap && !ctx->lists[lb].cap) continue;
        const double both = (double)std::max(ctx->lists[la].cap, ctx->lists[lb].cap);
        rc = ensure_list(ctx, la, 0, 0, both);
        if (!rc && ctx->lists[lb].cap) rc = ensure_list(ctx, lb, 0, 0, both);
    }
    if (rc) return finish_with(rc);
    int32_t zero = 0;
    if (hipMemcpyAsync(reinterpret_cast<char *>(ctx->st) + offsetof(DevState, done), &zero, sizeof(zero),
                       hipMemcpyHostToDevice, ctx->stream) != hipSuccess ||
        hipStreamSynchronize(ctx->stream) != hipSuccess)
        return finish_with(fail(ctx, CVO_HIP_ERR_HIP, "resume failed"));
    *ctx->done_mirror = 0;
    *ctx->progress_mirror = 0;
    *ctx->run_mirror = 0;
    *ctx->hint_mirror = -1;
    *ctx->side_mirror = 0;
    j.side_seen = 0;
    j.runs_enq = 0;
    j.run_waiting = false;
    j.spec_pending = false;
    if (hipMemset(reinterpret_cast<char *>(ctx->st) + offsetof(DevState, n_slots), 0, sizeof(int32_t)) != hipSuccess ||
        hipMemset(reinterpret_cast<char *>(ctx->st) + offsetof(DevState, run_count), 0, sizeof(int32_t)) != hipSuccess ||
        hipDeviceSynchronize() != hipSuccess)
        return finish_with(fail(ctx, CVO_HIP_ERR_HIP, "resume failed"));
    launch_prepare(ctx->st, loop_params(ctx), ctx->stream, ctx->table.raw ? ctx->table.masks() : nullptr);
    if (hipGetLastError() != hipSuccess) return finish_with(fail(ctx, CVO_HIP_ERR_HIP, "resume failed"));
    if (!ctx->profiling && !host_reduce(ctx)) {
        rc = prepare_lone_plan(ctx, j.trace_cap);
        if (rc) return finish_with(rc);
    }
    j.enq = j.batches = j.checked = 0;
    j.phase = 0;
    return 0;
}


}

extern "C" {

int cvo_hip_align(cvo_hip_ctx *ctx, cvo_hip_state *s, cvo_hip_trace *trace, int trace_cap,
                  int *n_iter)
{
    cvo_lock::Api api_guard;
    if (!ctx || !s) return CVO_HIP_ERR_INVALID;
    AlignJob j;
    j.ctx = ctx; j.s = s; j.trace = trace; j.trace_cap = trace_cap; j.n_iter = n_iter;
    j.paced = true;
    ctx->run_g_call = RUN_G;
    ctx->call_no_spec = false;
    int rc = job_begin(j);
    if (rc) return rc;
    while (!job_pump(j, true)) {}
    return j.rc;
}


}
```

cvo-rgbd_amd/csrc/cvo_kernels.hip:

```cpp
#include <algorithm>
#include <atomic>
#include <cstdlib>

#include "cvo_device.h"
#include "cvo_pair.h"

namespace cvo_dev {

typedef float f32x4 __attribute__((ext_vector_type(4)));

__device__ __forceinline__ float mv_row(const float *m, float x, float y, float z)
{
    return (m[0] * x + m[1] * y) + m[2] * z;
}

constexpr int FILTER_KMAX = 64;
size_t filter_smem_bytes(int jt)
{
    return (size_t)jt * 16 + ROWS_PER_TILE * 16 + 4 * TILE_STAGE * sizeof(TileEntry) +
           FILTER_KMAX * 4 * 4;
}

__device__ __forceinline__ void flush_tiles(const TileEntry *stage, int n, int lane, unsigned rot, unsigned region,
                                            const FilterArgs &a, int list, TileEntry *tiles, const int par)
// ... 1502 lines not shown
            if (dist < p.eps_2) {
                iter = k;
                done = DONE_BREAK_B;
                if (tr) tr->exit_code = 2;
            } else {
                if (acvo) {
                    ell = (float)((double)ell + p.dl_step * dl);
                    if (ell >= ell_max) {
                        ell = (float)(ell_max * 0.7);
                        ell_max = (float)(ell_max * 0.7);
                    }
                    ell = (ell < p.ell_min) ? p.ell_min : ell;
                } else {
                    ell = (k > 2) ? (float)0.10 : ell;
                    ell = (k > 9) ? (float)0.06 : ell;
                    ell = (k > 19) ? (float)0.03 : ell;
                }
                if (k + 1 >= p.max_iter) done = DONE_MAX_ITER;
                k = k + 1;
            }
        }
        if (timed) clk[2] = (long long)__builtin_readcyclecounter();
    }
    if (lane0) {
#pragma unroll
        for (int q = 0; q < 9; ++q) lds->R[q] = R[q];
#pragma unroll
        for (int q = 0; q < 3; ++q) lds->T[q] = T[q];
        lds->ell = ell; lds->ell_max = ell_max;
        lds->k = k; lds->iter = iter; lds->n_exec = n_exec; lds->n_slots = n_slots;
        lds->done = done;
        if (HM != HM_CLASSIC) lds->pending = 0;
    }
}

template <int HM>
__device__ __forceinline__ void head_plan(DevHead *lds, const PostStepArgs &a, const bool ran_post, const bool stalled,
                                          const unsigned (&flag)[LIST_N])
{
    const DevParams &p = a.prm;
    const bool async = p.async_xy != 0, aself = p.async_self != 0;
    const bool lane0 = (threadIdx.x & 63) == 0;
    PlanBuilds pb = HM == HM_CLASSIC ? plan_builds_classic(lds, false, false, false) : plan_builds_head(lds, false, false, false);
    pb.xy_failed = async && pb.xy_fresh >= 0 && (pb.xy_fresh ? flag[LIST_XYB] : flag[LIST_XY]) != 0u;
    pb.sf_failed[0] = aself ? (pb.sf_fresh[0] >= 0 && (pb.sf_fresh[0] ? flag[LIST_XXB] : flag[LIST_XX]) != 0u)
                            : (HM == HM_CLASSIC && stalled && flag[LIST_XX] != 0u);
    pb.sf_failed[1] = aself ? (pb.sf_fresh[1] >= 0 && (pb.sf_fresh[1] ? flag[LIST_YYB] : flag[LIST_YY]) != 0u)
                            : (HM == HM_CLASSIC && stalled && flag[LIST_YY] != 0u);
    const int xy_ck_done = (HM == HM_HEAD && ran_post && a.ck_nblk[LIST_XY] != 0 && flag[LIST_KEPT] == 0u) ? a.ck_nblk[LIST_XY] : 0;
    const int xy_ck_buf = lds->xy_active ? 1 : 0;
    const int sf_ck_done[2] = {(HM == HM_HEAD && ran_post && flag[LIST_KEPT] == 0u) ? a.ck_nblk[LIST_XX] : 0,
                               (HM == HM_HEAD && ran_post && flag[LIST_KEPT] == 0u) ? a.ck_nblk[LIST_YY] : 0};
    const int sf_ck_buf[2] = {lds->sf_active[0] ? 1 : 0, lds->sf_active[1] ? 1 : 0};
    bool ck_ok[3] = {false, false, false};
    if (HM == HM_CLASSIC && ran_post && flag[LIST_KEPT] == 0u) {
#pragma unroll
        for (int l = 0; l < 3; ++l) ck_ok[l] = a.ck_nblk[l] != 0 && flag[l] == 0u;
    }
    int done = lds->done;
    int pending = 0;
    {
        DevHead L;
        __builtin_memcpy(&L, lds, sizeof(DevHead));
        if (HM == HM_CLASSIC) {
            if (ck_ok[LIST_XY] && L.ck_nblk[LIST_XY] != a.ck_nblk[LIST_XY] && !p.async_xy) {
                if (L.reuse[LIST_XY]) L.list_stat[2] += 1;
                if (L.narrow & REC_BOUNDED) {
#pragma unroll
                    for (int q = 0; q < 9; ++q) { L.rec_Rt[q] = L.Rt[q]; if (lane0) lds->rec_Rt[q] = L.Rt[q]; }
#pragma unroll
                    for (int q = 0; q < 3; ++q) { L.rec_t[q] = L.t[q]; if (lane0) lds->rec_t[q] = L.t[q]; }
                }
            }
#pragma unroll
            for (int l = 0; l < 3; ++l)
                if (ck_ok[l]) L.ck_nblk[l] = a.ck_nblk[l];
        }
        if (xy_ck_done) { if (xy_ck_buf) L.xy_ck[1] = xy_ck_done; else L.xy_ck[0] = xy_ck_done; }
#pragma unroll
        for (int l = 0; l < 2; ++l)
            if (sf_ck_done[l]) { if (sf_ck_buf[l]) L.sf_ck[l][1] = sf_ck_done[l]; else L.sf_ck[l][0] = sf_ck_done[l]; }
        prepare_iteration(&L, lds, lane0, p, pb);
        if (pb.xy_failed || pb.sf_failed[0] || pb.sf_failed[1]) done = NEED_BIGGER_LIST;
        if (HM == HM_HEAD) pending = (done == RUNNING) ? 1 : 0;
        if (lane0) {
#pragma unroll
            for (int q = 0; q < 9; ++q) lds->Rt[q] = L.Rt[q];
#pragma unroll
            for (int q = 0; q < 3; ++q) { lds->t[q] = L.t[q]; lds->tauf[q] = L.tauf[q]; lds->list_r[q] = L.list_r[q];
                                          lds->list_ok[q] = L.list_ok[q]; lds->reuse[q] = L.reuse[q]; lds->ck_nblk[q] = L.ck_nblk[q]; }
            lds->kc_ell = L.kc_ell; lds->run_hint = L.run_hint; lds->r_last = L.r_last;
            lds->rec_r = L.rec_r; lds->narrow = L.narrow;
#pragma unroll
            for (int q = 0; q < 3; ++q) lds->list_stat[q] = L.list_stat[q];
            lds->xy_active = L.xy_active; lds->xy_target = L.xy_target; lds->stall = L.stall; lds->xy_fresh = L.xy_fresh;
            lds->tauf_build = L.tauf_build;
#pragma unroll
            for (int q = 0; q < 2; ++q) {
                lds->xy_ok[q] = L.xy_ok[q]; lds->xy_ck[q] = L.xy_ck[q]; lds->xy_r[q] = L.xy_r[q]; lds->rec_count[q] = L.rec_count[q];
                lds->sf_active[q] = L.sf_active[q]; lds->sf_target[q] = L.sf_target[q]; lds->sf_fresh[q] = L.sf_fresh[q];
                lds->sf_ok[q][0] = L.sf_ok[q][0]; lds->sf_ok[q][1] = L.sf_ok[q][1];
                lds->sf_ck[q][0] = L.sf_ck[q][0]; lds->sf_ck[q][1] = L.sf_ck[q][1];
                lds->sf_r[q][0] = L.sf_r[q][0]; lds->sf_r[q][1] = L.sf_r[q][1];
                lds->sf_tauf_build[q] = L.sf_tauf_build[q];
            }
            lds->done = done;
            if (HM != HM_CLASSIC) lds->pending = pending;
            count_async_plan(lds, lds, p);
        }
    }
}

template <int HM>
__device__ __forceinline__ void head_math(DevHead *lds, const PostStepArgs &a, const bool run_post, const bool stalled,
                                          const unsigned (&flag)[LIST_N], const bool publisher, const bool timed,
                                          long long (&clk)[4])
{
    head_post<HM>(lds, a, run_post, publisher, timed, clk);
    if (lds->done == RUNNING) head_plan<HM>(lds, a, run_post, stalled, flag);
    if (timed) clk[3] = (long long)__builtin_readcyclecounter();
}

template <int HM>
__device__ __forceinline__ void head_prepare_lists(const PostStepArgs &a, const DevHead *s_st)
{
    const int tid = threadIdx.x;
    const int nthr = blockDim.x;
    const bool async = a.prm.async_xy != 0, aself = a.prm.async_self != 0;
    if (a.build_mask && tid < 3) {
        const bool sync_list = !((async && tid == LIST_XY) || (aself && tid != LIST_XY));
        const bool build = sync_list && s_st->done == RUNNING && s_st->reuse[tid] == 0;
        if (build) atomicOr(&a.build_mask[tid], a.slot_bit);
        else atomicAnd(&a.build_mask[tid], ~a.slot_bit);
    }
    if (!(s_st->done == RUNNING || s_st->done == NEED_BIGGER_LIST)) return;
#pragma unroll
    for (int l = 0; l < 3; ++l) {
        if (s_st->reuse[l] || (async && l == LIST_XY) || (aself && l != LIST_XY)) continue;
        for (int q = tid; q < NSUB; q += nthr) a.st->sub[l][q] = 0u;
        if (tid == 0) atomicOr(&a.st->built[l][(s_st->k >> 5) & 63], 1u << (s_st->k & 31));
    }
    if (async && s_st->xy_target >= 0) {
        const int l = s_st->xy_target ? (int)LIST_XYB : (int)LIST_XY;
        for (int q = tid; q < NSUB; q += nthr) a.st->sub[l][q] = 0u;
    }
    if (aself)
        for (int l = 0; l < 2; ++l)
            if (s_st->sf_target[l] >= 0) {
                const int id = self_list_id(l, s_st->sf_target[l]);
                for (int q = tid; q < NSUB; q += nthr) a.st->sub[id][q] = 0u;
            }
    if (HM == HM_CLASSIC && tid < 8 && s_st->done == RUNNING) a.st->ovf[0][tid] = 0u;
}
__device__ __forceinline__ void head_publish(const PostStepArgs &a, const DevHead *s_st, DevHead *out, const bool math)
{
    const bool final_out = a.final_mirror != nullptr && (s_st->done == DONE_BREAK_A || s_st->done == DONE_BREAK_B || s_st->done == DONE_MAX_ITER);
    if (final_out) {
        const uint4 *src = reinterpret_cast<const uint4 *>(s_st);
        uint4 *dst = reinterpret_cast<uint4 *>(a.final_mirror);
        constexpr int pieces = (int)(DEVSTATE_HEAD_BYTES / 16);
        static_assert(pieces > 64 && pieces <= 128 && offsetof(DevHead, head_check_) == DEVSTATE_HEAD_BYTES - 12,
                      "one wave copies the head, two pieces per lane; the check word is the last piece's second word, held by the lanes' second pieces");
        if (threadIdx.x < 64) {
            const int p1 = (int)threadIdx.x + 64;
            const uint4 v0 = src[threadIdx.x];
            uint4 v = make_uint4(0u, 0u, 0u, 0u);
            if (p1 < pieces) v = src[p1];
            if (p1 == pieces - 1) v.y = 0u;
            unsigned sum = head_check_mix(v0.x, v0.y, v0.z, v0.w, threadIdx.x) + (p1 < pieces ? head_check_mix(v.x, v.y, v.z, v.w, (unsigned)p1) : 0u);
#pragma unroll
            for (int off = 32; off > 0; off >>= 1) sum += (unsigned)__shfl_xor((int)sum, off, 64);
            if (p1 == pieces - 1) v.y = sum;
            dst[threadIdx.x] = v0;
            if (p1 < pieces) dst[p1] = v;
        }
        __threadfence_system();
        __syncthreads();
    }
    if (threadIdx.x == 0) {
        if (math && a.hint_mirror && s_st->done == RUNNING) *a.hint_mirror = s_st->run_hint;
        if (math && a.progress_mirror && s_st->done == RUNNING) *a.progress_mirror = s_st->n_slots;
        if (a.done_mirror && s_st->done != RUNNING) *a.done_mirror = s_st->done;
    }
    state_head_from_lds(s_st, out);
}

template <int HM>
__device__ __forceinline__ bool head_body(const PostStepArgs &a, const DevHead *in, DevHead *out, DevHead *s_st,
                                          double *sh , const int par, const bool publisher,
                                          const ProcessArgs *count_pa = nullptr)
{
    const int tid = threadIdx.x;
    __shared__ unsigned s_cand_total;
    const bool count = HM == HM_HEAD && publisher && count_pa != nullptr && a.run_mail != nullptr && count_pa->cand_cnt != nullptr &&
                       count_pa->cand_cnt_b != nullptr;
    if (count && tid == 0) s_cand_total = 0u;
    const bool reduce = HM != HM_CLASSIC || (a.flags & POST_REDUCE) != 0;
    const bool math = HM != HM_CLASSIC || (a.flags & POST_MATH) != 0;
    const bool timed = a.dbg != nullptr && publisher;
    const long long c0 = timed ? (long long)__builtin_readcyclecounter() : 0;
    double sp[NACC_STEP];
    if (reduce) thread_load_partials<NACC_STEP>(a.part_step, a.nblk, sp);
    const unsigned my_flag = a.st->ovf[HM == HM_CLASSIC ? 0 : (par ^ 1)][tid & 7];
    state_head_to_lds(in, s_st);
    if (a.check_done && s_st->done != 0) {
        if (HM == HM_HEAD && publisher) state_head_from_lds(s_st, out);
        return false;
    }
    const bool async = a.prm.async_xy != 0;
    const bool stalled = async && s_st->stall != 0;
    const bool pending = HM == HM_CLASSIC ? true : (s_st->pending != 0);
    const bool run_post = pending && !stalled;
    const long long c1 = timed ? (long long)__builtin_readcyclecounter() : 0;
    if (reduce && run_post) block_finish_partials<NACC_STEP>(sp, sh, s_st->red + RED_STEP);
    const long long c2 = timed ? (long long)__builtin_readcyclecounter() : 0;
    bool comm_ok = true;
    if (HM == HM_CLASSIC && a.comm && !stalled) {
        __shared__ double sh_mail[MAX_WORLD * MAIL_VALS];
        __shared__ int sh_fail;
        comm_ok = mailbox_allreduce(*a.comm, a.st, s_st->red + RED_STEP, RED_N - RED_STEP, sh_mail, &sh_fail, s_st);
        if (!comm_ok && tid == 0) s_st->done = DONE_COMM_ERROR;
    }
    if (math && comm_ok) {
        const int act0 = s_st->xy_active ? 1 : 0;
        if (tid < 64) {
            unsigned flag[LIST_N];
#pragma unroll
            for (int l = 0; l < LIST_N; ++l) flag[l] = (unsigned)__builtin_amdgcn_readlane((int)my_flag, l);
            long long clk[4] = {0, 0, 0, 0};
            head_math<HM>(s_st, a, run_post, stalled, flag, publisher, timed, clk);
            if (timed && tid == 0 && run_post) {
                a.dbg[0] += 1; a.dbg[1] += c1 - c0; a.dbg[2] += c2 - c1;
                a.dbg[3] += clk[1] - clk[0]; a.dbg[4] += clk[2] - clk[1]; a.dbg[5] += clk[3] - clk[2];
                a.dbg[6] = c0;
            }
        } else if (count) {
            const uint32_t *c = act0 ? count_pa->cand_cnt_b : count_pa->cand_cnt;
            const unsigned wcap = count_pa->kept_wcap;
            const int nsl = 4 * count_pa->nblk;
            unsigned sum = 0u;
            for (int sl = tid - 64; sl < nsl; sl += BLOCK - 64) {
                const unsigned v = c[sl];
                sum += v < wcap ? v : wcap;
            }
#pragma unroll
            for (int off = 32; off > 0; off >>= 1) sum += (unsigned)__shfl_xor((int)sum, off, 64);
            if ((tid & 63) == 0) atomicAdd(&s_cand_total, sum);
        }
        __syncthreads();
        if (count) {
            if (tid == 0 && s_st->done == RUNNING && (s_st->xy_active ? 1 : 0) == act0 && (act0 ? s_st->xy_ck[1] : s_st->xy_ck[0]) == count_pa->nblk) {
                if (act0) s_st->rec_count[1] = (int32_t)s_cand_total; else s_st->rec_count[0] = (int32_t)s_cand_total;
                if (s_st->stall == 0 && s_st->xy_target < 0 && s_st->xy_fresh < 0) s_st->run_hint = (int32_t)s_cand_total;
            }
            __syncthreads();
        }
        if (publisher) head_prepare_lists<HM>(a, s_st);
    }
    if (publisher) head_publish(a, s_st, out, math);
    return s_st->done == RUNNING && !(async && s_st->stall != 0);
}

__device__ __forceinline__ void post_step_body(const PostStepArgs &a)
{
    __shared__ double sh[4 * NACC_MAX];
    __shared__ __attribute__((aligned(16))) DevHead s_st;
    head_body<HM_CLASSIC>(a, a.st, a.st, &s_st, sh, 0, true);
}

__global__ void __launch_bounds__(BLOCK) k_post_step(const Grp<PostStepArgs> grp)
{
    post_step_body(grp.a[blockIdx.z]);
}

__device__ __forceinline__ void prepare_body(DevState *st, const DevParams &prm, uint32_t *build_masks, const PrepareInit &init)
{
    if (init.on) {
        static_assert(DEVSTATE_INIT_BYTES % 4 == 0, "word stores");
        uint32_t *z = reinterpret_cast<uint32_t *>(st);
        for (int q = threadIdx.x; q < (int)(DEVSTATE_INIT_BYTES / 4); q += BLOCK) z[q] = 0u;
        __syncthreads();
        if (threadIdx.x == 0) {
            for (int q = 0; q < 9; ++q) st->R[q] = init.R[q];
            for (int q = 0; q < 3; ++q) { st->T[q] = init.T[q]; st->center[q] = init.center[q]; }
            st->ell = init.ell; st->ell_max = init.ell_max;
            st->iter = init.iter; st->n_fixed = init.n_fixed; st->done = init.done;
            st->xmax = init.xmax; st->y0max = init.y0max;
        }
        __syncthreads();
    }
    if (build_masks && threadIdx.x < 4) build_masks[threadIdx.x] = 0xffffffffu;
    for (int q = threadIdx.x; q < LIST_N * NSUB; q += BLOCK) (&st->sub[0][0])[q] = 0u;
    if (threadIdx.x < 16) (&st->ovf[0][0])[threadIdx.x] = 0u;
    if (threadIdx.x == 0) {
        for (int l = 0; l < 3; ++l) {
            st->list_ok[l] = 0;
            atomicOr(&st->built[l][(st->k >> 5) & 63], 1u << (st->k & 31));
        }
        for (int l = 0; l < 2; ++l) {
            st->sf_ok[l][0] = st->sf_ok[l][1] = 0;
            st->sf_ck[l][0] = st->sf_ck[l][1] = 0;
            st->sf_active[l] = 0; st->sf_target[l] = -1; st->sf_fresh[l] = -1;
        }
        st->xy_ok[0] = st->xy_ok[1] = 0;
        st->xy_ck[0] = st->xy_ck[1] = 0;
        st->rec_count[0] = st->rec_count[1] = 0;
        st->xy_active = 0;
        st->xy_target = -1;
        st->xy_fresh = -1;
        st->stall = 0;
        st->pending = 0;
        st->mail_snap = st->mail_seq;
        prepare_iteration(st, st, true, prm, plan_builds_none());
        count_async_plan(st, st, prm);
    }
}

__global__ void k_prepare(DevState *st, const DevParams prm, uint32_t *build_masks, const PrepareInit init)
{
    prepare_body(st, prm, build_masks, init);
}

__global__ void k_prepare_many(const Grp<PrepareEntry> grp, uint32_t *build_masks)
{
    const PrepareEntry &e = grp.a[blockIdx.x];
    prepare_body(e.st, e.prm, blockIdx.x == 0 ? build_masks : nullptr, e.init);
}

void launch_prepare(DevState *st, const DevParams &prm, hipStream_t s, uint32_t *build_masks, const PrepareInit *init)
{
    PrepareInit in{};
    if (init) in = *init;
    hipLaunchKernelGGL(k_prepare, dim3(1), dim3(BLOCK), 0, s, st, prm, build_masks, in);
}

void launch_prepare_many(const PrepareEntry *e, int n, hipStream_t s, uint32_t *build_masks)
{
    for (int at = 0; at < n; at += MAXG) {
        const int m = n - at < MAXG ? n - at : MAXG;
        Grp<PrepareEntry> g;
        for (int i = 0; i < m; ++i) g.a[i] = e[at + i];
        for (int i = m; i < MAXG; ++i) g.a[i] = e[at];
        hipLaunchKernelGGL(k_prepare_many, dim3((unsigned)m), dim3(BLOCK), 0, s, g, build_masks);
    }
}

void launch_post_flow_group(const PostFlowArgs *a, int n, hipStream_t s)
{
    Grp<PostFlowArgs> g;
    for (int i = 0; i < n; ++i) g.a[i] = a[i];
    hipLaunchKernelGGL(k_post_flow, dim3(1, 1, (unsigned)n), dim3(BLOCK), 0, s, g);
}

void launch_post_step_group(const PostStepArgs *a, int n, hipStream_t s)
{
    Grp<PostStepArgs> g;
    for (int i = 0; i < n; ++i) g.a[i] = a[i];
    hipLaunchKernelGGL(k_post_step, dim3(1, 1, (unsigned)n), dim3(BLOCK), 0, s, g);
}

typedef const __attribute__((address_space(4))) Slot *CSlot;
#define CVO_SLOT(tab)                          \
    CSlot cs = (CSlot)(tab) + blockIdx.z;      \
    if (cs->active == 0) return
#define CVO_ARG(T, field) (*(const T *)(&cs->field))
#define CVO_FILTER_ROLE(role) (*(const FilterArgs *)(&cs->op[q + (role)].f))

__global__ void __launch_bounds__(BLOCK) __attribute__((amdgpu_waves_per_eu(6, 8)))
kt_filter(const Slot *__restrict__ tab, const int ql)
{
    const int q = ql & QP_MASK, list = (ql >> 8) & 3;
    typedef const __attribute__((address_space(4))) uint32_t *CMask;
    const CMask masks = (CMask)(reinterpret_cast<const char *>(tab) - kTableHeaderBytes);
    const bool may_build = ((masks[list] >> blockIdx.z) & 1u) != 0u;
    constexpr unsigned PT_BLOCKS = 64;
    if (!may_build && blockIdx.x >= PT_BLOCKS) return;
    CVO_SLOT(tab);
    if (may_build) filter_body(CVO_ARG(FilterArgs, op[q].f), blockIdx.x, gridDim.x, cs->op[q].f.st, 0);
    if (blockIdx.x < PT_BLOCKS)
        pretransform_body(CVO_ARG(FilterArgs, op[q].f), blockIdx.x, min(gridDim.x, PT_BLOCKS));
}

__global__ void __launch_bounds__(BLOCK) __attribute__((amdgpu_waves_per_eu(6, 8)))
kt_filter_group(const Slot *__restrict__ tab, const int q)
{
    typedef const __attribute__((address_space(4))) uint32_t *CMask;
    const CMask masks = (CMask)(reinterpret_cast<const char *>(tab) - kTableHeaderBytes);
    const bool may_build = ((masks[blockIdx.y] >> blockIdx.z) & 1u) != 0u;
    constexpr unsigned PT_BLOCKS = 64;
    if (!may_build && (blockIdx.y != 0 || blockIdx.x >= PT_BLOCKS)) return;
    CVO_SLOT(tab);
    if (may_build) filter_body(CVO_FILTER_ROLE((int)blockIdx.y), blockIdx.x, gridDim.x, cs->op[q + (int)blockIdx.y].f.st, 0);
    if (blockIdx.y == 0 && blockIdx.x < PT_BLOCKS) pretransform_body(CVO_FILTER_ROLE(0), blockIdx.x, min(gridDim.x, PT_BLOCKS));
}

#ifndef CVO_FLOW_WAVES
#define CVO_FLOW_WAVES 5
#endif
template <int MODE, int WEIGHT = 0>
__global__ void __launch_bounds__(BLOCK) __attribute__((amdgpu_waves_per_eu((MODE == PROC_FLOW && WEIGHT == 0) ? CVO_FLOW_WAVES : 1, 8)))
kt_process(const Slot *__restrict__ tab, const int q)
{
    __shared__ __attribute__((aligned(16))) char scratch[PROC_SMEM];
    CVO_SLOT(tab);
    const ProcessArgs &a = CVO_ARG(ProcessArgs, op[q].p);
    ProcHead hd = proc_head_global<MODE>(a, a.st, 0);
    if (MODE == PROC_FLOW && WEIGHT == 0) hd.need_d2 = 0;
    process_body<MODE, WEIGHT>(a, blockIdx.x, scratch, hd);
}

__global__ void __launch_bounds__(BLOCK) kt_flow_d2(const Slot *__restrict__ tab, const int q)
{
    __shared__ __attribute__((aligned(16))) char scratch[PROC_SMEM];
    CVO_SLOT(tab);
    const ProcessArgs &a = CVO_ARG(ProcessArgs, op[q].p);
    process_body<PROC_FLOW, 0>(a, blockIdx.x, scratch, proc_head_global<PROC_FLOW>(a, a.st, 0));
}

__global__ void __launch_bounds__(BLOCK) kt_self2(const Slot *__restrict__ tab, const int q)
{
    __shared__ __attribute__((aligned(16))) char scratch[PROC_SMEM];
    CVO_SLOT(tab);
    const ProcessArgs &a = CVO_ARG(ProcessArgs, op[q + blockIdx.y].p);
    process_body<PROC_SELF>(a, blockIdx.x, scratch, proc_head_global<PROC_SELF>(a, a.st, 0));
}

__global__ void __launch_bounds__(STEP_BLOCK) kt_step_twist(const Slot *__restrict__ tab, const int qp)
{
    CSlot cs = (CSlot)(tab) + blockIdx.z;
    const int q = qp & QP_MASK, par = (qp & QP_PARITY) ? 1 : 0;
    const bool head_mode = (qp & QP_HEAD) != 0;
    const ProcessArgs &a = CVO_ARG(ProcessArgs, op[q].p);
    {
        const int active = cs->active;
        const int nblk = a.nblk, check_done = a.check_done, async_xy = a.async_xy, packed = a.kept_packed;
        const unsigned wcap = a.kept_wcap;
        const DevState *st = a.st, *st2 = a.st2;
        const double *fp = a.flow_part;
        const uint32_t *kc = a.kept_cnt;
        const uint2 *kij = a.kept_ij;
        const float *ka = a.kept_a;
        asm volatile("" ::"s"(active), "s"(nblk), "s"(check_done), "s"(async_xy), "s"(packed), "s"(wcap), "s"(st), "s"(st2),
                     "s"(fp), "s"(kc), "s"(kij), "s"(ka));
        if (active == 0) return;
    }
    DevState *const st_a = a.st, *const st_b = a.st2;
    step_twist_body(a, head_mode ? (par ? st_a : st_b) : st_a, par, head_mode);
}

__global__ void __launch_bounds__(BLOCK) kt_post_flow(const Slot *__restrict__ tab, const int q)
{
    CVO_SLOT(tab);
    const PostFlowArgs a = CVO_ARG(PostFlowArgs, op[q].pf);
    post_flow_body(a);
}

__global__ void __launch_bounds__(BLOCK) kt_post_step(const Slot *__restrict__ tab, const int q)
{
    CVO_SLOT(tab);
    const PostStepArgs a = CVO_ARG(PostStepArgs, op[q].ps);
    post_step_body(a);
}

#define CVO_MERGED_KERNELS(SUFFIX, WAVES)                                                                  \
    __global__ void __launch_bounds__(BLOCK) __attribute__((amdgpu_waves_per_eu(WAVES, 8)))               \
    kt_flow_build##SUFFIX(const Slot *__restrict__ tab, const int q)                                       \
    {                                                                                                      \
        extern __shared__ __attribute__((aligned(16))) char smem[];                                        \
        CVO_SLOT(tab);                                                                                     \
        const int np = cs->op[q].np;                                                                       \
        if ((int)blockIdx.x < np) {                                                                        \
            const ProcessArgs &pa = CVO_ARG(ProcessArgs, op[q].p);                                         \
            process_body<PROC_FLOW, 0, false, false>(pa, blockIdx.x, smem, proc_head_global<PROC_FLOW>(pa, pa.st, 0)); \
            return;                                                                                        \
        }                                                                                                  \
        filter_body<false>(CVO_ARG(FilterArgs, op[q].f), blockIdx.x - (unsigned)np, (unsigned)cs->op[q].n0,       \
                    cs->op[q].f.st, 0);                                                                    \
    }                                                                                                      \
    __global__ void __launch_bounds__(BLOCK) __attribute__((amdgpu_waves_per_eu(WAVES, 8)))               \
    kt_flow_build3##SUFFIX(const Slot *__restrict__ tab, const int q)                                      \
    {                                                                                                      \
        extern __shared__ __attribute__((aligned(16))) char smem[];                                        \
        CVO_SLOT(tab);                                                                                     \
        int b = (int)blockIdx.x;                                                                           \
        const int np = cs->op[q].np, n0 = cs->op[q].n0, n1 = cs->op[q].n1, n2 = cs->op[q].n2;             \
        if (b < np) {                                                                                      \
            const ProcessArgs &pa = CVO_ARG(ProcessArgs, op[q].p);                                         \
            process_body<PROC_FLOW, 0, false, false>(pa, (unsigned)b, smem, proc_head_global<PROC_FLOW>(pa, pa.st, 0)); \
            return;                                                                                        \
        }                                                                                                  \
        b -= np;                                                                                           \
        const int role = b < n0 ? 0 : (b < n0 + n1 ? 1 : 2);                                               \
        filter_body<false>(CVO_FILTER_ROLE(role), (unsigned)(b - (role == 0 ? 0 : (role == 1 ? n0 : n0 + n1))),   \
                    (unsigned)(role == 0 ? n0 : (role == 1 ? n1 : n2)), cs->op[q + role].f.st, 0);         \
    }                                                                                                      \
    __global__ void __launch_bounds__(BLOCK) __attribute__((amdgpu_waves_per_eu(WAVES, 8)))               \
    kt_flow_build6##SUFFIX(const Slot *__restrict__ tab, const int q)                                      \
    {                                                                                                      \
        extern __shared__ __attribute__((aligned(16))) char smem[];                                        \
        CVO_SLOT(tab);                                                                                     \
        int b = (int)blockIdx.x;                                                                           \
        const int np = cs->op[q].np;                                                                       \
        if (b < np) {                                                                                      \
            const ProcessArgs &pa = CVO_ARG(ProcessArgs, op[q].p);                                         \
            process_body<PROC_FLOW, 0, false, false>(pa, (unsigned)b, smem, proc_head_global<PROC_FLOW>(pa, pa.st, 0)); \
            return;                                                                                        \
        }                                                                                                  \
        b -= np;                                                                                           \
        if (b < 2 * np) {                                                                                  \
            const int w = b >= np ? 1 : 0;                                                                 \
            const ProcessArgs &pa = CVO_ARG(ProcessArgs, op[q + 1 + w].p);                                 \
               \
            process_body<PROC_SELF, 0, false, false>(pa, (unsigned)(b - w * np), smem, proc_head_global<PROC_SELF>(pa, pa.st, 0)); \
            return;                                                                                        \
        }                                                                                                  \
        b -= 2 * np;                                                                                       \
        const int n0 = cs->op[q].n0, n1 = cs->op[q].n1;                                                    \
        const int role = b < n0 ? 0 : (b < n0 + n1 ? 1 : 2);                                               \
        filter_body<false>(CVO_FILTER_ROLE(role), (unsigned)(b - (role == 0 ? 0 : (role == 1 ? n0 : n0 + n1))),   \
                    (unsigned)(role == 0 ? n0 : (role == 1 ? n1 : cs->op[q].n2)), cs->op[q + role].f.st, 0); \
    }
CVO_MERGED_KERNELS(_w4, 4)

template <int MODE>
__device__ __forceinline__ ProcHead proc_head_lds(const ProcessArgs &a, const DevHead *h, const int par, float (&rt)[12])
{
    auto uni = [](float x) { return __int_as_float(__builtin_amdgcn_readfirstlane(__float_as_int(x))); };
    auto unid = [](double x) {
        return __hiloint2double(__builtin_amdgcn_readfirstlane(__double2hiint(x)), __builtin_amdgcn_readfirstlane(__double2loint(x)));
    };
    ProcHead hd;
#pragma unroll
    for (int q = 0; q < 9; ++q) rt[q] = uni(h->Rt[q]);
#pragma unroll
    for (int q = 0; q < 3; ++q) rt[9 + q] = uni(h->t[q]);
    hd.Rt = rt; hd.tt = rt + 9; hd.xi = nullptr;
    const KernConsts &k = h->kc;
    hd.kc.tau = uni(k.tau); hd.kc.tau_c = uni(k.tau_c); hd.kc.sp = uni(k.sp);
    hd.kc.inv_c = uni(k.inv_c); hd.kc.inv_d = uni(k.inv_d); hd.kc.inv_l3 = uni(k.inv_l3);
    hd.kc.cb = uni(k.cb); hd.kc.cg = uni(k.cg); hd.kc.cd = uni(k.cd); hd.kc.cscale = uni(k.cscale);
    hd.kc.s2_d = unid(k.s2_d); hd.kc.cs2_d = unid(k.cs2_d);
    hd.kc.ninv_2l2 = unid(k.ninv_2l2); hd.kc.ninv_2cl2 = unid(k.ninv_2cl2);
    hd.done_word = 0;
    hd.n_fixed = (MODE == PROC_SELF && a.first_counted) ? __builtin_amdgcn_readfirstlane(h->n_fixed) : 0;
    hd.second = ((MODE == PROC_FLOW && __builtin_amdgcn_readfirstlane(h->xy_active) == 1) ||
                 (MODE == PROC_SELF && __builtin_amdgcn_readfirstlane(h->sf_active[a.async_self == 2 ? 1 : 0]) == 1)) ? 1 : 0;
    hd.list_bad = 0u;
    hd.ck_nblk = 0;
    hd.par = par;
    hd.cand = nullptr; hd.cand_cnt = nullptr;
    hd.need_d2 = a.need_d2;
    hd.narrow = 0; hd.rec_lim = PAD_BIG;
    if (a.cand_b) {
        const int l = a.async_self == 2 ? 1 : 0;
        const int ck = MODE == PROC_FLOW ? (hd.second ? h->xy_ck[1] : h->xy_ck[0]) : (hd.second ? h->sf_ck[l][1] : h->sf_ck[l][0]);
        hd.ck_nblk = __builtin_amdgcn_readfirstlane(ck);
        hd.cand = hd.second ? a.cand_b : a.cand;
        hd.cand_cnt = hd.second ? a.cand_cnt_b : a.cand_cnt;
    }
    return hd;
}

#define CVO_SLOT_HEAD(tab)                                                                                    \
    CSlot cs = (CSlot)(tab) + blockIdx.z;                                                                     \
    const int q = qp & QP_MASK, par = (qp & QP_PARITY) ? 1 : 0;                                               \
    {                                                                                                         \
        const PostStepArgs &hps = CVO_ARG(PostStepArgs, op[q].ps);                                            \
        const int active = cs->active, np_ = cs->op[q].np, hn = hps.nblk, hcd = hps.check_done;               \
        const DevState *hst = hps.st, *hst2 = hps.st2;                                                        \
        const double *hpart = hps.part_step;                                                                  \
        const long long *hdbg = hps.dbg;                                                                      \
        asm volatile("" ::"s"(active), "s"(np_), "s"(hn), "s"(hcd), "s"(hst), "s"(hst2), "s"(hpart), "s"(hdbg)); \
        if (active == 0) return;                                                                              \
    }
#define CVO_HEAD_KERNELS(SUFFIX, WAVES)                                                                    \
    __global__ void __launch_bounds__(BLOCK) __attribute__((amdgpu_waves_per_eu(WAVES, 8)))               \
    kt_hflow_build##SUFFIX(const Slot *__restrict__ tab, const int qp)                                     \
    {                                                                                                      \
        extern __shared__ __attribute__((aligned(16))) char smem[];                                        \
        __shared__ double sh[4 * NACC_MAX];                                                                \
        __shared__ __attribute__((aligned(16))) DevHead s_st;                                              \
        CVO_SLOT_HEAD(tab);                                                                                \
        const int np = cs->op[q].np;                                                                       \
        if ((int)blockIdx.x >= np) {                                                                       \
            const FilterArgs &f = CVO_ARG(FilterArgs, op[q].f);                                            \
            filter_body<false>(f, blockIdx.x - (unsigned)np, (unsigned)cs->op[q].n0, par ? f.st2 : f.st, par);    \
            return;                                                                                        \
        }                                                                                                  \
        const PostStepArgs ps = CVO_ARG(PostStepArgs, op[q].ps);                                           \
        const ProcessArgs &pa = CVO_ARG(ProcessArgs, op[q].p);                                             \
        if (!head_body<HM_HEAD>(ps, par ? ps.st2 : ps.st, par ? ps.st : ps.st2, &s_st, sh, par,            \
                                blockIdx.x == 0, &pa)) return;                                             \
        float rt[12];                                                                                      \
        process_body<PROC_FLOW, 0, true, false>(pa, blockIdx.x, smem, proc_head_lds<PROC_FLOW>(pa, &s_st, par, rt)); \
        if (ps.dbg && blockIdx.x == 0 && threadIdx.x == 0 && ps.dbg[6] != 0) {    \
            ps.dbg[7] += (long long)__builtin_readcyclecounter() - ps.dbg[6];                              \
            ps.dbg[6] = 0;                                                                                 \
        }                                                                                                  \
    }                                                                                                      \
    __global__ void __launch_bounds__(BLOCK) __attribute__((amdgpu_waves_per_eu(WAVES, 8)))               \
    kt_hflow_build6##SUFFIX(const Slot *__restrict__ tab, const int qp)                                    \
    {                                                                                                      \
        extern __shared__ __attribute__((aligned(16))) char smem[];                                        \
        __shared__ double sh[4 * NACC_MAX];                                                                \
        __shared__ __attribute__((aligned(16))) DevHead s_st;                                              \
        CVO_SLOT_HEAD(tab);                                                                                \
        int b = (int)blockIdx.x;                                                                           \
        const int np = cs->op[q].np;                                                                       \
        if (b >= 3 * np) {                                                                                 \
            b -= 3 * np;                                                                                   \
            const int n0 = cs->op[q].n0, n1 = cs->op[q].n1;                                                \
            const int role = b < n0 ? 0 : (b < n0 + n1 ? 1 : 2);                                           \
            const FilterArgs &f = CVO_FILTER_ROLE(role);                                                   \
            filter_body<false>(f, (unsigned)(b - (role == 0 ? 0 : (role == 1 ? n0 : n0 + n1))),                   \
                        (unsigned)(role == 0 ? n0 : (role == 1 ? n1 : cs->op[q].n2)), par ? f.st2 : f.st, par); \
            return;                                                                                        \
        }                                                                                                  \
        const PostStepArgs ps = CVO_ARG(PostStepArgs, op[q].ps);                                           \
        const int role = b < np ? 0 : (b < 2 * np ? 1 : 2);                             \
        const unsigned rb = (unsigned)(b - role * np);                                                     \
        const ProcessArgs &pa = CVO_ARG(ProcessArgs, op[q + role].p);                                      \
        if (!head_body<HM_HEAD>(ps, par ? ps.st2 : ps.st, par ? ps.st : ps.st2, &s_st, sh, par,            \
                                blockIdx.x == 0)) return;                                                  \
        float rt[12];                                                                                      \
        if (role == 0) {                                                                                   \
            process_body<PROC_FLOW, 0, true, false>(pa, rb, smem, proc_head_lds<PROC_FLOW>(pa, &s_st, par, rt));  \
            return;                                                                                        \
        }                                                                                                  \
        process_body<PROC_SELF, 0, true, false>(pa, rb, smem, proc_head_lds<PROC_SELF>(pa, &s_st, par, rt));      \
    }
CVO_HEAD_KERNELS(_w4, 4)


constexpr long long RUN_TIMEOUT_TICKS = 100000000LL;
enum { RUN_V_STALL = 1, RUN_V_BUILD = 2, RUN_V_RELOAD = 4 };
enum { RUN_GO = 1, RUN_ABORT = 2 };
constexpr long long RUN_ENTRY_TICKS = 20000LL;

struct RunNoWork { __device__ __forceinline__ void operator()() const {} };
#ifndef CVO_RUN_POLL_GAP
#define CVO_RUN_POLL_GAP 0
#endif
#ifndef CVO_RUN_POLL_SLEEP
#define CVO_RUN_POLL_SLEEP 1
#endif
template <int K, class SRC>
__device__ __forceinline__ bool run_poll(const SRC &src, const unsigned tag, const long long timeout_ticks, unsigned long long (&w)[K], int *s_fail)
{
    const unsigned long long none = (unsigned long long)tag << 32;
    auto sweep = [&](unsigned long long (&v)[K]) {
#pragma unroll
        for (int k = 0; k < K; ++k) {
            const unsigned long long *p = src(k);
            v[k] = p ? __hip_atomic_load(p, __ATOMIC_RELAXED, __HIP_MEMORY_SCOPE_AGENT) : none;
        }
    };
    auto in = [&](const unsigned long long (&v)[K]) {
        bool ok = true;
#pragma unroll
        for (int k = 0; k < K; ++k) ok = ok && (unsigned)(v[k] >> 32) == tag;
        return ok;
    };
    const long long t0 = (long long)wall_clock64();
    if (CVO_RUN_POLL_GAP == 0) {
        for (;;) {
            sweep(w);
            if (in(w)) return true;
            if ((long long)wall_clock64() - t0 > timeout_ticks) { *s_fail = 1; return false; }
            __builtin_amdgcn_s_sleep(CVO_RUN_POLL_SLEEP);
        }
    }
    unsigned long long b[K];
    sweep(w);
    __builtin_amdgcn_s_sleep(CVO_RUN_POLL_GAP);
    sweep(b);
    for (;;) {
        if (in(w)) return true;
        if ((long long)wall_clock64() - t0 > timeout_ticks) { *s_fail = 1; return false; }
        sweep(w);
        if (in(b)) {
#pragma unroll
            for (int k = 0; k < K; ++k) w[k] = b[k];
            return true;
        }
        sweep(b);
    }
}
template <int NV, int KMAX, class AFTER>
__device__ __forceinline__ bool run_exchange_k(RunMail *mail, const int row, const int g, const unsigned long long seq, const double my_val,
                                             double *all , double *part , double *tot ,
                                             int *s_fail, unsigned *verdict_out, unsigned *s_verdict, const long long timeout_ticks, const AFTER &after_post)
{
    const int tid = threadIdx.x;
    const unsigned tag = (unsigned)seq;
    unsigned long long *slot = &mail->w[seq & (unsigned long long)(RUN_GEN - 1)][0][0];
    if (row >= 0 && tid < 2 * NV) {
        const unsigned long long bits = (unsigned long long)__double_as_longlong(my_val);
        const unsigned half = (tid & 1) ? (unsigned)(bits >> 32) : (unsigned)bits;
        __hip_atomic_store(&slot[row * (2 * RUN_NV) + tid], ((unsigned long long)tag << 32) | half, __ATOMIC_RELAXED,
                           __HIP_MEMORY_SCOPE_AGENT);
    }
    after_post();
    const int nrow = g * 2 * NV, nwords = nrow + (verdict_out ? 1 : 0);
    if constexpr (KMAX <= 2) {
        unsigned long long w[KMAX];
        auto src = [&](const int k) -> const unsigned long long * {
            const int wi = tid + k * RUN_BLOCK;
            if (wi >= nwords) return nullptr;
            const int r = wi / (2 * NV), c = wi - r * (2 * NV);
            return wi == nrow ? &mail->w[(seq >> 1) & 1ull][RUN_G][0] : &slot[r * (2 * RUN_NV) + c];
        };
        if (run_poll<KMAX>(src, tag, timeout_ticks, w, s_fail)) {
#pragma unroll
            for (int k = 0; k < KMAX; ++k) {
                const int wi = tid + k * RUN_BLOCK;
                if (wi < nrow) reinterpret_cast<unsigned *>(all)[wi] = (unsigned)w[k];
                else if (wi == nrow && verdict_out) *s_verdict = (unsigned)w[k];
            }
        }
    } else
    {
// ... 1165 lines not shown
```

Before: 4413 registrations/s.

## Let tail registrations leave fused engine early via host-signaled device flag

Adds a tail_early mode, on by default. During wind-down the host sets a pinned-memory leave flag that the post-step kernel polls. A still-running registration then stores its state, marks its slot as left so later batched kernels skip it, and publishes a DONE_LEFT_ENGINE verdict. The host picks these jobs up and resumes them alone right away instead of waiting for the engine batch to drain, which targets idle tail time. This adds device-host polling, spin-waiting on the host and extra state-handover logic, with a risk of races in the slot-left protocol.

After: 4367 registrations/s. -1.0%, worse.

```diff
diff --git a/cvo-rgbd_amd/csrc/cvo_capi.cpp b/cvo-rgbd_amd/csrc/cvo_capi.cpp
--- a/cvo-rgbd_amd/csrc/cvo_capi.cpp
+++ b/cvo-rgbd_amd/csrc/cvo_capi.cpp
@@ -42,6 +42,7 @@
     {"engine_crowd", "CVO_HIP_ENGINE_CROWD", 2, 0.0},     {"engine_merge_max", "CVO_HIP_ENGINE_MERGE_MAX", 2, 0.0},
     {"matches_combine", nullptr, 0, 0.0},                 {"scan_chunk", nullptr, 0, 0.0},
     {"record_narrow", "CVO_HIP_NO_RECORD_NARROW", 1, 0.0}, {"list_stale_max", "CVO_HIP_LIST_STALE_MAX", 2, 0.0},
+    {"tail_early", "CVO_HIP_NO_TAIL_EARLY", 1, 0.0},
 };
 void env_defaults(cvo_hip_ctx *ctx)
 {
@@ -102,6 +103,7 @@
     else if (is("wait_policy")) { if (v < 0.0 || v > 2.0) return CVO_HIP_ERR_INVALID; o.wait_policy = (int)v; }
     else if (is("acvo_runs")) o.no_acvo_run = !on;
     else if (is("tail_alone")) { if (v < 0.0 || v > 32.0) return CVO_HIP_ERR_INVALID; o.tail_alone = (int)v; }
+    else if (is("tail_early")) o.tail_early = on;
     else if (is("run_restart")) o.no_restart = !on;
     else if (is("side_builds")) o.no_side_builds = !on;
     else if (is("run_build_at")) { if (!(v > 0.0 && v <= 1.0)) return CVO_HIP_ERR_INVALID; o.run_build_at = (float)v; }
@@ -857,7 +859,11 @@
     else if (is("wait_policy")) *value = o.wait_policy;
     else if (is("acvo_runs")) *value = !o.no_acvo_run;
     else if (is("tail_alone")) *value = o.tail_alone;
+    else if (is("tail_early")) *value = o.tail_early;
     else if (is("tail_handovers")) *value = (double)ctx->tail_handovers;
+    else if (is("tail_left_early")) *value = (double)ctx->tail_left_early;
+    else if (is("tail_left_backstop")) *value = (double)ctx->tail_left_backstop;
+    else if (is("tail_gap_us")) *value = ctx->tail_gap_us;
     else if (is("run_restart")) *value = !o.no_restart;
     else if (is("side_builds")) *value = !o.no_side_builds;
     else if (is("run_build_at")) *value = o.run_build_at;
diff --git a/cvo-rgbd_amd/csrc/cvo_device.h b/cvo-rgbd_amd/csrc/cvo_device.h
--- a/cvo-rgbd_amd/csrc/cvo_device.h
+++ b/cvo-rgbd_amd/csrc/cvo_device.h
@@ -45,7 +45,8 @@
 
 enum { RUNNING = 0, DONE_BREAK_A = 1, DONE_BREAK_B = 2, DONE_MAX_ITER = 3, NEED_BIGGER_LIST = 4,
        DONE_COMM_ERROR = 5,
-       DONE_RUN_TIMEOUT = 6 };
+       DONE_RUN_TIMEOUT = 6,
+       DONE_LEFT_ENGINE = 7 };
 
 constexpr int MAX_WORLD = 16;
 constexpr int MAIL_VALS = 14;
@@ -307,6 +308,9 @@
     int32_t *side_mirror;
     float run_build_at;
     int run_fault;
+    const int32_t *leave;
+    int32_t *left;
+    int leave_from;
     DevParams prm;
 };
 
@@ -323,7 +327,8 @@
 };
 struct Slot {
     int active;
-    int pad_[3];
+    int left;
+    int pad_[2];
     OpArgs op[MAX_OPS];
 };
 
diff --git a/cvo-rgbd_amd/csrc/cvo_engine.cpp b/cvo-rgbd_amd/csrc/cvo_engine.cpp
--- a/cvo-rgbd_amd/csrc/cvo_engine.cpp
+++ b/cvo-rgbd_amd/csrc/cvo_engine.cpp
@@ -65,6 +65,13 @@
     bool narrow_merge = false;
     int narrow_blocks = 0;
     bool wind_down = false;
+    int32_t *leave = nullptr;
+    long long sync_mark = 0;
+    bool asked = false;
+    bool may_ask() const { return checked >= sync_mark; }
+    bool tail_early = false;
+    int leave_from = 0;
+    long long n_left_early = 0, n_left_backstop = 0;
     std::vector<TLaunch> plan;
     struct FlowEv { hipEvent_t a, b; int live; };
     std::vector<FlowEv> flow_ev;
@@ -78,6 +85,8 @@
         if (hipSetDevice(dev) != hipSuccess) return -1;
         if (hipStreamCreateWithFlags(&s, hipStreamNonBlocking) != hipSuccess) return -1;
         if (tab.init(ENGINE_SLOTS, s) != 0) return -1;
+        if (hipHostMalloc((void **)&leave, 64, hipHostMallocDefault) != hipSuccess) { leave = nullptr; return -1; }
+        *leave = 0;
         for (auto &e : ev)
             if (hipEventCreateWithFlags(&e, hipEventDisableTiming) != hipSuccess) return -1;
         return 0;
@@ -220,8 +229,21 @@
         if (!plan_fused(po, ps, zdim, plan)) return CVO_HIP_ERR_INVALID;
         for (int z = 0; z < ENGINE_SLOTS; ++z)
             if (member[z]) set_build_masks(slot[z], plan, tab.masks(), z);
+        if (tail_early && leave)
+            for (int z = 0; z < ENGINE_SLOTS; ++z) {
+                if (!member[z]) continue;
+                for (const TLaunch &l : plan) {
+                    if (l.kernel != TK_POST_STEP) continue;
+                    PostStepArgs &ps = slot[z].op[l.q].ps;
+                    if (!ps.final_mirror) continue;
+                    ps.leave = leave;
+                    ps.left = &tab.dev[z].left;
+                    ps.leave_from = leave_from;
+                }
+            }
         const int nq = po.empty() ? 0 : (int)po[0]->size();
         if (tab.sync(slot, s, nq) != 0) return CVO_HIP_ERR_HIP;
+        sync_mark = launched;
         ++n_replans;
         dirty = false;
         return CVO_HIP_OK;
@@ -235,7 +257,7 @@
             if (!j) continue;
             cvo_hip_ctx *c = j->ctx;
             const int32_t verdict = *(volatile int32_t *)c->done_mirror;
-            if (verdict == RUNNING) continue;
+            if (verdict == RUNNING || verdict == DONE_LEFT_ENGINE) continue;
             const bool mirrored = (verdict == DONE_BREAK_A || verdict == DONE_BREAK_B || verdict == DONE_MAX_ITER) && c->final_mirror &&
                                   !c->opt.no_final_mirror && !multi_rank(c);
             if (mirrored && take_final_mirror(c, verdict)) {
@@ -338,6 +360,11 @@
             { const double t0 = now_ms(); collect_stopped(); t_collect += now_ms() - t0; }
             moved = true;
         }
+        if (wind_down && tail_early) {
+            const int before = live();
+            if (before > 0) { const double t0 = now_ms(); collect_stopped(); t_collect += now_ms() - t0; }
+            if (live() != before) moved = true;
+        }
         { const double t0 = now_ms(); if (finish_arrived(pending, false)) moved = true; t_finish += now_ms() - t0; }
         while (!wind_down && !pending.empty() && live() < std::min(want, (int)ENGINE_SLOTS)) {
             AlignJob *j = pending.front();
@@ -387,6 +414,25 @@
             AlignJob *j = member[z];
             if (!j) continue;
             out.push_back(j);
+            ++n_left_backstop;
+            ++j->ctx->tail_left_backstop;
+            member[z] = nullptr;
+            ops[z].clear();
+            dirty = true;
+        }
+    }
+
+    void take_early(std::vector<AlignJob *> &out)
+    {
+        if (!wind_down || !tail_early || failed) return;
+        for (int z = 0; z < ENGINE_SLOTS; ++z) {
+            AlignJob *j = member[z];
+            if (!j) continue;
+            cvo_hip_ctx *c = j->ctx;
+            if (*(volatile int32_t *)c->done_mirror != DONE_LEFT_ENGINE || !c->final_mirror || !take_final_mirror(c, DONE_LEFT_ENGINE)) continue;
+            out.push_back(j);
+            ++n_left_early;
+            ++c->tail_left_early;
             member[z] = nullptr;
             ops[z].clear();
             dirty = true;
@@ -456,13 +502,14 @@
     std::lock_guard<std::mutex> lock(*engine_mutex());
     if (engine_debug_on())
         fprintf(stderr, "[cvo_hip] engine %p: batches at zdim 1/2/4/8/16: %lld %lld %lld %lld %lld, replans %lld, "
-                "prepare launches %lld, final states mirrored %lld copied %lld, graph captures %lld hits %lld; host ms: insert %.2f replan %.2f launch %.2f collect %.2f finish %.2f wait %.2f\n",
+                "prepare launches %lld, final states mirrored %lld copied %lld, left early %lld by the backstop %lld, graph captures %lld hits %lld; host ms: insert %.2f replan %.2f launch %.2f collect %.2f finish %.2f wait %.2f\n",
                 (void *)e, e->n_batches[0], e->n_batches[1], e->n_batches[2],
-                e->n_batches[3], e->n_batches[4], e->n_replans, e->n_prepares, e->n_mirrored, e->n_copied, e->plans.captures, e->plans.hits,
+                e->n_batches[3], e->n_batches[4], e->n_replans, e->n_prepares, e->n_mirrored, e->n_copied, e->n_left_early, e->n_left_backstop, e->plans.captures, e->plans.hits,
                 e->t_insert, e->t_replan, e->t_launch, e->t_collect, e->t_finish, e->t_wait);
     e->t_insert = e->t_replan = e->t_launch = e->t_collect = e->t_finish = e->t_wait = 0;
     for (long long &v : e->n_batches) v = 0;
     e->n_replans = e->n_prepares = e->n_mirrored = e->n_copied = 0;
+    e->n_left_early = e->n_left_backstop = 0;
     e->launched = e->checked = 0;
     e->in_use = false;
 }
@@ -491,6 +538,21 @@
     int first_err = CVO_HIP_OK;
     std::vector<char> taken((size_t)count, 0);
     std::vector<AlignJob *> leavers;
+    std::vector<char> cont((size_t)count, 0), begun((size_t)count, 0);
+    std::vector<int> early;
+    double tail_gap_ms = -1.0;
+    auto start_alone = [&](int i, int share, bool resume) {
+        int cus = 0;
+        if (hipDeviceGetAttribute(&cus, hipDeviceAttributeMultiprocessorCount, jobs[i].ctx->device) != hipSuccess || cus <= 0) cus = RUN_G + 8;
+        jobs[i].ctx->run_g_call = share > 1 ? std::max(8, (cus - 8) / share - 1) : RUN_G;
+        jobs[i].ctx->call_no_spec = share > 2;
+        jobs[i].ctx->crowded = false;
+        jobs[i].ctx->lone = true;
+        jobs[i].paced_nb = true;
+        begun[(size_t)i] = 1;
+        const int rc = resume ? job_continue_alone(jobs[i]) : job_begin(jobs[i]);
+        if (rc) { jobs[i].rc = rc; jobs[i].phase = 2; if (!first_err) first_err = rc; }
+    };
     const bool no_fuse = count > 0 && ctxs[0] && ctxs[0]->opt.no_fuse;
     if (!no_fuse && count > 1) {
         constexpr int gmax = ENGINE_SLOTS;
@@ -544,6 +606,17 @@
                           (double)c->fixed.n * (double)c->moving.n <= 2.0e8;
             }
             const bool narrow_merge_ok = !pending.empty() && (pending.front()->ctx->opt.narrow_merge || pending.front()->ctx->opt.narrow_blocks > 0) && !engine_profile()->on;
+            const bool tail_early = tail_ok && !pending.empty() && pending.front()->ctx->opt.tail_early;
+            for (Engine *e : engines) {
+                e->tail_early = tail_early;
+                e->asked = false;
+                e->sync_mark = 0;
+                e->leave_from = narrow_from;
+                __atomic_store_n(e->leave, 0, __ATOMIC_RELEASE);
+            }
+            int tail_share = 1;
+            double t_wind = 0.0;
+            std::vector<AlignJob *> early_now;
             int dbg_left = -1, dbg_narrow = -1;
             for (;;) {
                 bool any = false, moved = false;
@@ -565,6 +638,9 @@
                     (void)settled;
                     if (tail_ok && left > 0 && left <= tail_k && narrow) {
                         for (Engine *e : engines) e->wind_down = true;
+                        tail_share = left;
+                        t_wind = Engine::now_ms();
+                        tail_gap_ms = std::max(tail_gap_ms, 0.0);
                         if (dbg_many) {
                             fprintf(stderr, "[cvo_hip]   tail: %d registrations left after %.2f ms, slots done:", left, Engine::now_ms() - t_many0);
                             for (Engine *e : engines)
@@ -576,13 +652,39 @@
                 }
                 for (Engine *e : engines) {
                     if (e->wind_down) {
+                        if (e->tail_early && !e->asked && !e->failed && e->live() > 0 && e->may_ask()) {
+                            __atomic_store_n(e->leave, 1, __ATOMIC_RELEASE);
+                            e->asked = true;
+                            if (dbg_many) fprintf(stderr, "[cvo_hip]   tail: engine %p asks its members to leave after %.2f ms\n", (void *)e, Engine::now_ms() - t_many0);
+                        }
+                        early_now.clear();
+                        e->take_early(early_now);
+                        for (AlignJob *j : early_now) {
+                            const int i = (int)(j - &jobs[0]);
+                            early.push_back(i);
+                            cont[(size_t)i] = 1;
+                            if (dbg_many) fprintf(stderr, "[cvo_hip]   tail: job %d leaves early at slot %d\n", i, jobs[i].ctx->st_host[0].n_slots);
+                            start_alone(i, tail_share, true);
+                            moved = true;
+                        }
+                        if (!early_now.empty()) {
+                            tail_gap_ms = std::max(tail_gap_ms, Engine::now_ms() - t_wind);
+                            if (dbg_many) fprintf(stderr, "[cvo_hip]   tail: %zu registrations leave engine %p early after %.2f ms\n", early_now.size(), (void *)e, Engine::now_ms() - t_many0);
+                        }
                         const size_t before = leavers.size();
                         e->release_members(leavers);
                         if (leavers.size() != before) {
                             moved = true;
+                            tail_gap_ms = std::max(tail_gap_ms, Engine::now_ms() - t_wind);
+                            for (size_t k = before; tail_early && k < leavers.size(); ++k) {
+                                const int i = (int)(leavers[k] - &jobs[0]);
+                                early.push_back(i);
+                                start_alone(i, tail_share, true);
+                            }
                             if (dbg_many) fprintf(stderr, "[cvo_hip]   tail: %zu registrations leave engine %p after %.2f ms\n", leavers.size() - before, (void *)e, Engine::now_ms() - t_many0);
                         }
                         while (!pending.empty()) {
+                            ++pending.front()->ctx->tail_left_backstop;
                             leavers.push_back(pending.front());
                             pending.pop_front();
                             moved = true;
@@ -595,43 +697,51 @@
                         fprintf(stderr, "[cvo_hip]   engine %p idle after %.2f ms\n", (void *)e, e->t_idle_at - t_many0);
                     }
                 }
+                int early_live = 0;
+                for (const int i : early) {
+                    if (jobs[i].phase == 2) continue;
+                    const int before_phase = jobs[i].phase, before_checked = jobs[i].checked + jobs[i].batches;
+                    if (job_pump(jobs[i], false)) {
+                        if (jobs[i].rc && !first_err) first_err = jobs[i].rc;
+                        moved = true;
+                        continue;
+                    }
+                    ++early_live;
+                    if (jobs[i].phase != before_phase || jobs[i].checked + jobs[i].batches != before_checked) moved = true;
+                }
                 if (!any && pending.empty()) break;
                 bool alive = false;
                 for (Engine *e : engines) alive = alive || !e->failed;
                 if (!alive) break;
-                if (!moved)
+                if (!moved) {
+                    bool watch = early_live > 0;
+                    for (Engine *e : engines) watch = watch || (e->wind_down && e->tail_early && !e->failed && e->live() > 0);
+                    if (watch) { __builtin_ia32_pause(); continue; }
                     for (Engine *e : engines)
                         if (!e->idle() && !e->failed) { e->wait_oldest(pending); break; }
-            }
-            for (Engine *e : engines) { e->wind_down = false; e->narrow = false; e->batch_len = kEngineBatch; engine_release(e); }
+                }
+            }
+            for (Engine *e : engines) {
+                __atomic_store_n(e->leave, 0, __ATOMIC_RELEASE);
+                e->wind_down = false; e->tail_early = false; e->asked = false; e->sync_mark = 0; e->narrow = false; e->batch_len = kEngineBatch;
+                engine_release(e);
+            }
         }
         for (int i = 0; i < count; ++i)
             if (jobs[i].phase == 2 && jobs[i].rc && !first_err) first_err = jobs[i].rc;
     }
-    std::vector<char> cont((size_t)count, 0);
     for (AlignJob *j : leavers) {
         const size_t i = (size_t)(j - &jobs[0]);
         taken[i] = 0;
         cont[i] = 1;
     }
+    for (const int i : early) taken[(size_t)i] = 0;
+    if (count > 0 && ctxs[0]) ctxs[0]->tail_gap_us = tail_gap_ms < 0.0 ? -1.0 : tail_gap_ms * 1e3;
     int k_alone = 0;
     for (int i = 0; i < count; ++i)
         if (!taken[i] && jobs[i].phase != 2) ++k_alone;
     const int kAloneLive = std::max<int>(8, (int)leavers.size());
-    std::vector<char> begun((size_t)count, 0);
-    auto begin_job = [&](int i) {
-        int cus = 0;
-        if (hipDeviceGetAttribute(&cus, hipDeviceAttributeMultiprocessorCount, jobs[i].ctx->device) != hipSuccess || cus <= 0) cus = RUN_G + 8;
-        const int share = std::min(k_alone, kAloneLive);
-        jobs[i].ctx->run_g_call = share > 1 ? std::max(8, (cus - 8) / share - 1) : RUN_G;
-        jobs[i].ctx->call_no_spec = share > 2;
-        jobs[i].ctx->crowded = false;
-        jobs[i].ctx->lone = true;
-        jobs[i].paced_nb = true;
-        begun[(size_t)i] = 1;
-        const int rc = cont[(size_t)i] ? job_continue_alone(jobs[i]) : job_begin(jobs[i]);
-        if (rc) { jobs[i].rc = rc; jobs[i].phase = 2; if (!first_err) first_err = rc; }
-    };
+    auto begin_job = [&](int i) { start_alone(i, std::min(k_alone, kAloneLive), cont[(size_t)i] != 0); };
     auto is_alone = [&](int i) { return !taken[i]; };
     for (;;) {
         int live = 0, moved = 0, first_live = -1, waiting = 0;
diff --git a/cvo-rgbd_amd/csrc/cvo_internal.h b/cvo-rgbd_amd/csrc/cvo_internal.h
--- a/cvo-rgbd_amd/csrc/cvo_internal.h
+++ b/cvo-rgbd_amd/csrc/cvo_internal.h
@@ -215,6 +215,7 @@
     bool no_restart = false;
     bool no_acvo_run = false;
     int tail_alone = 8;
+    bool tail_early = true;
     int alone_max = 0;
     int engines_force = 0;
     int narrow_blocks = 0;
@@ -237,6 +238,9 @@
     int no_run_backoff = 0;
     long long side_builds_launched = 0;
     long long tail_handovers = 0;
+    long long tail_left_early = 0;
+    long long tail_left_backstop = 0;
+    double tail_gap_us = -1.0;
     long long engine_begins = 0;
     long long engine_final_mirrored = 0;
     long long engine_final_copied = 0;
diff --git a/cvo-rgbd_amd/csrc/cvo_job.cpp b/cvo-rgbd_amd/csrc/cvo_job.cpp
--- a/cvo-rgbd_amd/csrc/cvo_job.cpp
+++ b/cvo-rgbd_amd/csrc/cvo_job.cpp
@@ -336,6 +336,8 @@
         }
         {
             const int32_t verdict = *(volatile int32_t *)ctx->done_mirror;
+            if (verdict == DONE_LEFT_ENGINE)
+                return finish_with(fail(ctx, CVO_HIP_ERR_HIP, "a launch of the engine a registration had left reached it again"));
             const bool mirrored = (verdict == DONE_BREAK_A || verdict == DONE_BREAK_B || verdict == DONE_MAX_ITER) && ctx->final_mirror &&
                                   ctx->table.image.size() == 1 && ctx->plan_has_final_mirror;
             if (mirrored && take_final_mirror(ctx, verdict)) return finish_with(job_finish(j));
diff --git a/cvo-rgbd_amd/csrc/cvo_kernels.hip b/cvo-rgbd_amd/csrc/cvo_kernels.hip
--- a/cvo-rgbd_amd/csrc/cvo_kernels.hip
+++ b/cvo-rgbd_amd/csrc/cvo_kernels.hip
@@ -1678,9 +1678,10 @@
             }
     if (HM == HM_CLASSIC && tid < 8 && s_st->done == RUNNING) a.st->ovf[0][tid] = 0u;
 }
-__device__ __forceinline__ void head_publish(const PostStepArgs &a, const DevHead *s_st, DevHead *out, const bool math)
-{
-    const bool final_out = a.final_mirror != nullptr && (s_st->done == DONE_BREAK_A || s_st->done == DONE_BREAK_B || s_st->done == DONE_MAX_ITER);
+__device__ __forceinline__ void head_publish(const PostStepArgs &a, const DevHead *s_st, DevHead *out, const bool math, const bool stored = false)
+{
+    const bool final_out = a.final_mirror != nullptr && (s_st->done == DONE_BREAK_A || s_st->done == DONE_BREAK_B || s_st->done == DONE_MAX_ITER ||
+                                                         s_st->done == DONE_LEFT_ENGINE);
     if (final_out) {
         const uint4 *src = reinterpret_cast<const uint4 *>(s_st);
         uint4 *dst = reinterpret_cast<uint4 *>(a.final_mirror);
@@ -1706,9 +1707,10 @@
     if (threadIdx.x == 0) {
         if (math && a.hint_mirror && s_st->done == RUNNING) *a.hint_mirror = s_st->run_hint;
         if (math && a.progress_mirror && s_st->done == RUNNING) *a.progress_mirror = s_st->n_slots;
-        if (a.done_mirror && s_st->done != RUNNING) *a.done_mirror = s_st->done;
-    }
-    state_head_from_lds(s_st, out);
+        if (stored && a.done_mirror) __hip_atomic_store(a.done_mirror, s_st->done, __ATOMIC_RELAXED, __HIP_MEMORY_SCOPE_SYSTEM);
+        else if (a.done_mirror && s_st->done != RUNNING) *a.done_mirror = s_st->done;
+    }
+    if (!stored) state_head_from_lds(s_st, out);
 }
 
 template <int HM>
@@ -1721,6 +1723,9 @@
     const bool count = HM == HM_HEAD && publisher && count_pa != nullptr && a.run_mail != nullptr && count_pa->cand_cnt != nullptr &&
                        count_pa->cand_cnt_b != nullptr;
     if (count && tid == 0) s_cand_total = 0u;
+    __shared__ int s_leave_req;
+    const bool may_leave = HM == HM_CLASSIC && publisher && a.leave != nullptr && a.left != nullptr && a.final_mirror != nullptr;
+    bool leaving = false;
     const bool reduce = HM != HM_CLASSIC || (a.flags & POST_REDUCE) != 0;
     const bool math = HM != HM_CLASSIC || (a.flags & POST_MATH) != 0;
     const bool timed = a.dbg != nullptr && publisher;
@@ -1772,8 +1777,11 @@
 #pragma unroll
             for (int off = 32; off > 0; off >>= 1) sum += (unsigned)__shfl_xor((int)sum, off, 64);
             if ((tid & 63) == 0) atomicAdd(&s_cand_total, sum);
+        } else if (may_leave && tid == BLOCK - 1) {
+            s_leave_req = __hip_atomic_load(a.leave, __ATOMIC_RELAXED, __HIP_MEMORY_SCOPE_SYSTEM);
         }
         __syncthreads();
+        if (may_leave) leaving = s_leave_req != 0 && s_st->done == RUNNING && s_st->n_slots >= a.leave_from;
         if (count) {
             if (tid == 0 && s_st->done == RUNNING && (s_st->xy_active ? 1 : 0) == act0 && (act0 ? s_st->xy_ck[1] : s_st->xy_ck[0]) == count_pa->nblk) {
                 if (act0) s_st->rec_count[1] = (int32_t)s_cand_total; else s_st->rec_count[0] = (int32_t)s_cand_total;
@@ -1783,7 +1791,15 @@
         }
         if (publisher) head_prepare_lists<HM>(a, s_st);
     }
-    if (publisher) head_publish(a, s_st, out, math);
+    if (leaving) {
+        state_head_from_lds(s_st, out);
+        if (tid == 0) *a.left = 1;
+        __threadfence_system();
+        __syncthreads();
+        if (tid == 0) s_st->done = DONE_LEFT_ENGINE;
+        __syncthreads();
+    }
+    if (publisher) head_publish(a, s_st, out, math, leaving);
     return s_st->done == RUNNING && !(async && s_st->stall != 0);
 }
 
@@ -1888,7 +1904,7 @@
 typedef const __attribute__((address_space(4))) Slot *CSlot;
 #define CVO_SLOT(tab)                          \
     CSlot cs = (CSlot)(tab) + blockIdx.z;      \
-    if (cs->active == 0) return
+    if ((cs->active == 0) | (cs->left != 0)) return
 #define CVO_ARG(T, field) (*(const T *)(&cs->field))
 #define CVO_FILTER_ROLE(role) (*(const FilterArgs *)(&cs->op[q + (role)].f))
 
@@ -1958,7 +1974,7 @@
     const bool head_mode = (qp & QP_HEAD) != 0;
     const ProcessArgs &a = CVO_ARG(ProcessArgs, op[q].p);
     {
-        const int active = cs->active;
+        const int active = (cs->active != 0) & (cs->left == 0);
         const int nblk = a.nblk, check_done = a.check_done, async_xy = a.async_xy, packed = a.kept_packed;
         const unsigned wcap = a.kept_wcap;
         const DevState *st = a.st, *st2 = a.st2;
@@ -2092,7 +2108,7 @@
     const int q = qp & QP_MASK, par = (qp & QP_PARITY) ? 1 : 0;                                               \
     {                                                                                                         \
         const PostStepArgs &hps = CVO_ARG(PostStepArgs, op[q].ps);                                            \
-        const int active = cs->active, np_ = cs->op[q].np, hn = hps.nblk, hcd = hps.check_done;               \
+        const int active = (cs->active != 0) & (cs->left == 0), np_ = cs->op[q].np, hn = hps.nblk, hcd = hps.check_done; \
         const DevState *hst = hps.st, *hst2 = hps.st2;                                                        \
         const double *hpart = hps.part_step;                                                                  \
         const long long *hdbg = hps.dbg;                                                                      \
```
